# floswald/SMM.jl

Hardware: AMD Instinct MI355X
Metric: chain-evals/sec (whole node), serialNormal 2p/2m, 4096 chains x 200 iters (higher is better)
Workload: dtype f64

## Files before the change

### include/smmhip.h

```cpp
#ifndef SMMHIP_H
#define SMMHIP_H

#include <stdint.h>

#ifdef __cplusplus
extern "C" {
#endif

#define SMMHIP_ABI_VERSION 3

#define SMM_REDUCE_LANES 512

typedef enum {
    SMM_OK = 0,
    SMM_ERR_INVALID_ARG = -1,
    SMM_ERR_NO_DEVICE = -2,
    SMM_ERR_NEGATIVE_OBJECTIVE = -3,
    SMM_ERR_NO_DRAW_IN_SUPPORT = -4,
    SMM_ERR_BAD_BATCH = -5,
    SMM_ERR_MAXITER = -6,
    SMM_ERR_HIP = -7,
    SMM_ERR_STATE = -8,
    SMM_ERR_EXCHANGE_CAPACITY = -9
} smm_status_t;
// ... 382 lines not shown
typedef struct {
    double*  best;
    double*  value;
    double*  sim_moments;
    double*  simplex;
    double*  simplex_value;
    double*  size_x;
    double*  size_f;
    int32_t* iterations;
    int32_t* status;
    int32_t* moves;
    int32_t* n_eval;
    int64_t  evaluated;
} smm_opt_simplex_t;
int  smm_opt_simplex(void* ctx, const double* starts , int32_t K, double step, int32_t adaptive, double xatol, double fatol,
                     int32_t max_iter, smm_opt_simplex_t* out);

typedef struct {
    double*  best;
    double*  value;
    double*  sim_moments;
    double*  ssr;
    double*  grad;
    double*  jac;
    double*  lambda;
    double*  step;
    double*  dF;
    int32_t* active;
    int32_t* iterations;
    int32_t* tries;
    int32_t* n_eval;
    int32_t* status;
    int64_t  evaluated;
} smm_opt_lm_t;
int  smm_opt_lm(void* ctx, const double* starts , int32_t K, double fd_step, double lambda0, double lambda_up,
                double lambda_down, double xtol, double ftol, double gtol, int32_t max_iter, int32_t max_tries, smm_opt_lm_t* out);

typedef struct {
    double*  theta;
    double*  value;
    double*  sim_moments;
    double*  weight;
    double*  logw;
    int32_t* born;
    double*  eps;
    double*  p_acc;
    double*  gen_ess;
    int32_t* n_outside;
    int32_t* n_invalid;
    int32_t* n_underflow;
    int32_t* n_new_kept;
    double*  mean;
    double*  cov;
    double*  quantile;
    double   ess;
    int32_t  n_kept;
    int32_t  generations;
    int32_t  status;
    int32_t  reserved;
    int64_t  evaluated;
} smm_abc_pmc_t;
int  smm_abc_pmc(void* ctx, int32_t n_particles , int32_t n_keep , int32_t max_gen, double p_acc_min, double scale ,
                 double ridge, const double* probs, int32_t n_probs, smm_abc_pmc_t* out);

typedef struct {
    double*  mean;
    double*  var;
    double*  centre;
    double*  first;
    double*  total;
    double*  v_first;
    double*  v_total;
    double*  se_first;
    double*  se_total;
    int64_t  n_complete;
    int64_t  n_invalid;
    int64_t  evaluated;
} smm_sens_sobol_t;
int  smm_sens_sobol(void* ctx, int32_t n_base , const double* lo, const double* hi , smm_sens_sobol_t* out);
int  smm_get_timing(void* ctx, smm_timing_t* out);
int  smm_set_profiling(void* ctx, int32_t on);
int  smm_set_persistent(void* ctx, int32_t on);
int  smm_get_persistent(void* ctx, int32_t* available, int32_t* launches, int32_t* repairs);
int  smm_describe(void* ctx, char* out, int32_t cap);
int  smm_get_Z(void* ctx, double* Z);

#ifdef __cplusplus
}
#endif
#endif
```

### smm.jl_amd/_abi.py

```python
import ctypes as C
import os

import numpy as np

_HERE = os.path.dirname(os.path.abspath(__file__))
LIB_PATH = os.path.join(_HERE, "csrc", "libsmmhip.so")
HOOKS_LIB_PATH = os.path.join(_HERE, "csrc", "libsmmhip_hooks.so")

c_double_p = C.POINTER(C.c_double)
c_int32_p = C.POINTER(C.c_int32)
c_uint8_p = C.POINTER(C.c_uint8)
c_int8_p = C.POINTER(C.c_int8)

SMM_OK = 0
SMM_ERR_INVALID_ARG = -1
SMM_ERR_NO_DEVICE = -2
SMM_ERR_NEGATIVE_OBJECTIVE = -3
SMM_ERR_NO_DRAW_IN_SUPPORT = -4
SMM_ERR_BAD_BATCH = -5
SMM_ERR_MAXITER = -6
SMM_ERR_HIP = -7
SMM_ERR_STATE = -8
SMM_ERR_EXCHANGE_CAPACITY = -9

# ... 214 lines not shown
    ]


SYMBOLS = [
    ("smm_abi_version", C.c_int, []),
    ("smm_register_user_objective", C.c_int, [C.c_char_p, C.POINTER(C.c_int32)]),
    ("smm_register_user_objective_lanes", C.c_int, [C.c_char_p, C.c_int32, C.c_int32, C.POINTER(C.c_int32)]),
    ("smm_register_user_objective_rng", C.c_int, [C.c_char_p, C.c_int32, C.c_int32, C.POINTER(C.c_int32)]),
    ("smm_device_count", C.c_int, []),
    ("smm_ctx_create", C.c_int, [C.POINTER(smm_problem_t), C.POINTER(smm_bgp_opts_t), C.POINTER(smm_tables_t),
                                 C.POINTER(C.c_void_p)]),
    ("smm_ctx_destroy", None, [C.c_void_p]),
    ("smm_last_error", C.c_char_p, [C.c_void_p]),
    ("smm_bgp_step", C.c_int, [C.c_void_p, C.c_int32]),
    ("smm_bgp_step_async", C.c_int, [C.c_void_p, C.c_int32]),
    ("smm_sync", C.c_int, [C.c_void_p]),
    ("smm_bgp_local_step", C.c_int, [C.c_void_p]),
    ("smm_bgp_record_doubles", C.c_int, [C.c_void_p]),
    ("smm_bgp_export_records_dev", C.c_int, [C.c_void_p, C.c_void_p]),
    ("smm_bgp_exchange_dev", C.c_int, [C.c_void_p, C.c_void_p]),
    ("smm_bgp_a2a_capacity", C.c_int, [C.c_void_p]),
    ("smm_bgp_export_values_dev", C.c_int, [C.c_void_p, C.c_void_p]),
    ("smm_bgp_a2a_pack_dev", C.c_int, [C.c_void_p, C.c_void_p, C.c_void_p]),
    ("smm_bgp_a2a_apply_dev", C.c_int, [C.c_void_p, C.c_void_p]),
    ("smm_bgp_sharded_step", C.c_int, [C.c_void_p, C.c_void_p, C.c_void_p]),
    ("smm_bgp_sharded_finish", C.c_int, [C.c_void_p, C.c_void_p]),
    ("smm_bgp_p2p_init", C.c_int, [C.c_void_p, C.c_void_p, C.POINTER(C.c_void_p)]),
    ("smm_bgp_p2p_attach", C.c_int, [C.c_void_p, C.c_int32, C.c_void_p, C.c_void_p]),
    ("smm_bgp_p2p_step", C.c_int, [C.c_void_p, C.c_int32]),
    ("smm_bgp_p2p_finish", C.c_int, [C.c_void_p]),
    ("smm_stream", C.c_void_p, [C.c_void_p]),
    ("smm_eval_batch", C.c_int, [C.c_void_p, c_double_p, C.c_int32, c_double_p, c_double_p, c_int8_p]),
    ("smm_eval_batch_noseed", C.c_int, [C.c_void_p, c_double_p, C.c_int32, C.c_uint64, c_double_p, c_double_p, c_int8_p]),
    ("smm_get_history", C.c_int, [C.c_void_p, C.c_int32, C.c_int32, C.POINTER(smm_history_t)]),
    ("smm_get_chain_stats", C.c_int, [C.c_void_p, C.c_int32, C.c_int32, C.c_int32, c_double_p, C.c_int32,
                                      C.POINTER(smm_chain_stats_t)]),
    ("smm_get_chain_diag", C.c_int, [C.c_void_p, C.c_int32, C.c_int32, C.c_int32, C.c_int32, c_int32_p, C.c_int32,
                                     C.POINTER(smm_chain_diag_t)]),
    ("smm_get_group_stats", C.c_int, [C.c_void_p, C.c_int32, C.c_int32, C.c_int32, c_int32_p, C.c_int32, c_double_p, C.c_int32,
                                      C.POINTER(smm_group_stats_t)]),
    ("smm_get_histogram", C.c_int, [C.c_void_p, C.c_int32, C.c_int32, C.c_int32, c_int32_p, C.c_int32, C.c_int32, c_double_p, c_int32_p,
                                     C.c_int32, C.c_int32, C.POINTER(smm_histogram_t)]),
    ("smm_get_trace", C.c_int, [C.c_void_p, C.c_int32, C.c_int32, C.c_int32, C.c_int32, C.c_int32, c_int32_p, C.c_int32, c_double_p, C.c_int32,
                                C.POINTER(smm_trace_t)]),
    ("smm_get_rank_diag", C.c_int, [C.c_void_p, C.c_int32, C.c_int32, C.c_int32, C.c_int32, c_int32_p, C.c_int32,
                                    C.POINTER(smm_rank_diag_t)]),
    ("smm_get_draws", C.c_int, [C.c_void_p, C.c_int32, C.c_int32, C.c_int32, c_int32_p, C.c_int32, C.c_int32, C.c_int32, C.c_int64,
                                C.POINTER(smm_draws_t)]),
    ("smm_get_moment_stats", C.c_int, [C.c_void_p, C.c_int32, C.c_int32, C.c_int32, c_int32_p, C.c_int32, c_double_p, C.c_int32, C.c_double,
                                       C.POINTER(smm_moment_stats_t)]),
    ("smm_get_adjustment", C.c_int, [C.c_void_p, C.c_int32, C.c_int32, C.c_int32, c_int32_p, C.c_int32, C.c_double, C.c_int32, c_double_p,
                                     C.c_double, c_double_p, C.c_int32, C.POINTER(smm_adjustment_t)]),
    ("smm_get_reweighted", C.c_int, [C.c_void_p, C.c_int32, C.c_int32, C.c_int32, c_int32_p, C.c_int32, c_double_p, C.c_int32, c_double_p,
                                     C.c_int32, C.POINTER(smm_reweighted_t)]),
    ("smm_get_profile", C.c_int, [C.c_void_p, C.c_int32, C.c_int32, C.c_int32, c_int32_p, C.c_int32, C.c_int32, c_double_p, c_int32_p,
                                   C.c_int32, C.c_int32, C.POINTER(smm_profile_t)]),
    ("smm_get_density", C.c_int, [C.c_void_p, C.c_int32, C.c_int32, C.c_int32, c_int32_p, C.c_int32, c_double_p, C.c_int32, C.c_int32,
                                   c_double_p, c_double_p, C.POINTER(smm_density_t)]),
    ("smm_register_user_transform", C.c_int, [C.c_char_p, C.c_int32, C.POINTER(C.c_int32)]),
    ("smm_get_derived", C.c_int, [C.c_void_p, C.c_int32, C.c_int32, C.c_int32, C.c_int32, c_int32_p, C.c_int32, c_double_p, C.c_int32,
                                   c_double_p, C.c_int32, C.POINTER(smm_derived_t)]),
    ("smm_get_chain_cov", C.c_int, [C.c_void_p, C.c_int32, C.c_int32, C.c_int32, C.c_int32, c_int32_p, c_double_p, c_double_p]),
    ("smm_get_proposal", C.c_int, [C.c_void_p, c_double_p]),
    ("smm_set_proposal", C.c_int, [C.c_void_p, c_double_p]),
    ("smm_adapt_proposal", C.c_int, [C.c_void_p, C.c_int32, C.c_int32, C.c_int32, C.c_int32, C.c_int32, C.c_double, c_int32_p]),
    ("smm_get_state", C.c_int, [C.c_void_p, C.POINTER(smm_state_t)]),
    ("smm_set_state", C.c_int, [C.c_void_p, C.POINTER(smm_state_t), C.POINTER(smm_history_t)]),
    ("smm_set_population", C.c_int, [C.c_void_p, c_double_p, C.POINTER(smm_population_t)]),
    ("smm_scatter_population", C.c_int, [C.c_void_p, C.c_int32, C.c_double, C.c_int32, C.POINTER(smm_population_t)]),
    ("smm_opt_slices", C.c_int, [C.c_void_p, c_double_p, C.c_int32, C.c_int32, C.c_double, C.c_double, C.c_int32,
                                 C.POINTER(smm_opt_slices_t)]),
    ("smm_opt_simplex", C.c_int, [C.c_void_p, c_double_p, C.c_int32, C.c_double, C.c_int32, C.c_double, C.c_double, C.c_int32,
                                  C.POINTER(smm_opt_simplex_t)]),
    ("smm_opt_lm", C.c_int, [C.c_void_p, c_double_p, C.c_int32, C.c_double, C.c_double, C.c_double, C.c_double, C.c_double, C.c_double,
                             C.c_double, C.c_int32, C.c_int32, C.POINTER(smm_opt_lm_t)]),
    ("smm_abc_pmc", C.c_int, [C.c_void_p, C.c_int32, C.c_int32, C.c_int32, C.c_double, C.c_double, C.c_double, c_double_p, C.c_int32,
                              C.POINTER(smm_abc_pmc_t)]),
    ("smm_sens_sobol", C.c_int, [C.c_void_p, C.c_int32, c_double_p, c_double_p, C.POINTER(smm_sens_sobol_t)]),
    ("smm_get_timing", C.c_int, [C.c_void_p, C.POINTER(smm_timing_t)]),
    ("smm_get_Z", C.c_int, [C.c_void_p, c_double_p]),
    ("smm_set_profiling", C.c_int, [C.c_void_p, C.c_int32]),
    ("smm_set_persistent", C.c_int, [C.c_void_p, C.c_int32]),
    ("smm_get_persistent", C.c_int, [C.c_void_p, C.POINTER(C.c_int32), C.POINTER(C.c_int32), C.POINTER(C.c_int32)]),
    ("smm_describe", C.c_int, [C.c_void_p, C.c_char_p, C.c_int32]),
]


class SMMHipError(RuntimeError):
    def __init__(self, code, msg):
        super().__init__("smmhip error %d: %s" % (code, msg))
        self.code = code


def bind(lib, symbols=SYMBOLS, prefix_from="smm_", prefix_to=None):
    for name, res, args in symbols:
        n = name if prefix_to is None else prefix_to + name[len(prefix_from):]
        fn = getattr(lib, n)
        fn.restype = res
        fn.argtypes = args
    return lib


_lib = None


def load():
    global _lib
    if _lib is None:
        path = LIB_PATH
        if not os.path.exists(path):
            raise ImportError(
                "libsmmhip.so not found at %s — build it with `python -c 'import __graft_entry__ as g; g.build()'` "
                "(hipcc --offload-arch=gfx950). There is no CPU fallback." % path)
        _lib = bind(C.CDLL(path, mode=C.RTLD_GLOBAL))
        if _lib.smm_abi_version() != 3:
            raise ImportError("libsmmhip.so ABI version mismatch")
    return _lib


_hooks_lib = None


def load_hooks():
    global _hooks_lib
    if _hooks_lib is None:
        if not os.path.exists(HOOKS_LIB_PATH):
            raise ImportError("libsmmhip_hooks.so not found at %s — `make -C smm.jl_amd/csrc all`" % HOOKS_LIB_PATH)
        lib = bind(C.CDLL(HOOKS_LIB_PATH, mode=C.RTLD_GLOBAL))
        lib.smm_debug_has_test_hooks.restype = C.c_int
        if lib.smm_abi_version() != 3 or lib.smm_debug_has_test_hooks() != 1:
            raise ImportError("libsmmhip_hooks.so: wrong ABI version or built without -DSMM_TEST_HOOKS")
        lib.smm_debug_user_form.restype = C.c_int
        lib.smm_debug_user_form.argtypes = [C.c_int32, C.c_int, C.POINTER(C.c_ulonglong), C.POINTER(C.c_ulonglong), C.c_char_p, C.c_int]
        _hooks_lib = lib
    return _hooks_lib


def use_test_hooks(on=True):
    global _lib
    _lib = load_hooks() if on else None
    return load()


def dptr(a):
    return None if a is None else a.ctypes.data_as(c_double_p)


def f64(a, shape=None):
    a = np.ascontiguousarray(a, dtype=np.float64)
    if shape is not None:
        assert a.shape == tuple(shape), (a.shape, shape)
    return a


class HistoryBuffers:

    def __init__(self, nt, N, np_, nm):
        self.value = np.empty((nt, N)); self.prob = np.empty((nt, N))
        self.curr_val = np.empty((nt, N)); self.best_val = np.empty((nt, N))
        self.params = np.empty((nt, np_, N)); self.sim_moments = np.empty((nt, nm, N))
        self.best_id = np.empty((nt, N), np.int32); self.exchanged = np.empty((nt, N), np.int32)
        self.accepted = np.empty((nt, N), np.uint8); self.status = np.empty((nt, N), np.int8)

    FIELDS = ("value", "prob", "curr_val", "best_val", "params", "sim_moments", "best_id", "exchanged", "accepted",
              "status")

# ... 29 lines not shown
```

### smm.jl_amd/backend.py

```python
import builtins as _builtins
import ctypes as C

import numpy as np

from . import _abi as A


class Problem:

    def __init__(self, init, lb, ub, mom, w=None, ns=10000, objective_id=A.SMM_OBJ_NORM, obj_params=None):
        self.init = A.f64(init); self.lb = A.f64(lb); self.ub = A.f64(ub)
        self.mom = A.f64(mom)
        self.w = A.f64(np.full(len(self.mom), np.nan) if w is None else w)
        self.np = len(self.init); self.nm = len(self.mom); self.ns = int(ns)
        self.objective_id = int(objective_id)
        self.obj_params = None if obj_params is None else A.f64(obj_params)
        assert len(self.lb) == self.np and len(self.ub) == self.np and len(self.w) == self.nm

    def struct(self):
        p = A.smm_problem_t()
        p.np, p.nm, p.ns, p.objective_id = self.np, self.nm, self.ns, self.objective_id
        p.init, p.lb, p.ub, p.mom, p.w = map(A.dptr, (self.init, self.lb, self.ub, self.mom, self.w))
        p.obj_params = A.dptr(self.obj_params)
        p.n_obj_params = 0 if self.obj_params is None else len(self.obj_params)
# ... 529 lines not shown
                 converged=np.empty(K, np.int32))
        s = self._out(A.smm_opt_slices_t, r)
        self._check(self._fn("opt_slices")(self._ctx, A.dptr(st), K, int(npoints), float(tol), float("nan") if update is None else float(update),
                                           int(max_cycles), C.byref(s)))
        r["evaluated"] = int(s.evaluated)
        return r

    def opt_simplex(self, starts, step=0.05, adaptive=False, xatol=1e-4, fatol=1e-4, max_iter=None):
        st, K = self._opt_starts("opt_simplex", starts)
        V = self.np + 1
        r = dict(best=np.empty((self.np, K)), value=np.empty(K), sim_moments=np.empty((self.nm, K)), simplex=np.empty((V, self.np, K)),
                 simplex_value=np.empty((V, K)), size_x=np.empty(K), size_f=np.empty(K), iterations=np.empty(K, np.int32),
                 status=np.empty(K, np.int32), moves=np.empty((5, K), np.int32), n_eval=np.empty(K, np.int32))
        s = self._out(A.smm_opt_simplex_t, r)
        self._check(self._fn("opt_simplex")(self._ctx, A.dptr(st), K, float(step), int(bool(adaptive)), float(xatol), float(fatol),
                                            200 * self.np if max_iter is None else int(max_iter), C.byref(s)))
        r["evaluated"] = int(s.evaluated)
        return r

    def opt_lm(self, starts, fd_step=1e-4, lambda0=1e-3, lambda_up=10, lambda_down=10, xtol=1e-8, ftol=1e-12, gtol=0.0, max_iter=100,
               max_tries=12):
        st, K = self._opt_starts("opt_lm", starts)
        i32 = lambda *shape: np.empty(shape, np.int32)
        r = dict(best=np.empty((self.np, K)), value=np.empty(K), sim_moments=np.empty((self.nm, K)), ssr=np.empty(K), grad=np.empty((self.np, K)),
                 jac=np.empty((self.nm, self.np, K)), step=np.empty(K), dF=np.empty(K), active=i32(self.np, K), iterations=i32(K), tries=i32(K),
                 n_eval=i32(K), status=i32(K))
        r["lambda"] = np.empty(K)
        s = self._out(A.smm_opt_lm_t, r)
        self._check(self._fn("opt_lm")(self._ctx, A.dptr(st), K, float(fd_step), float(lambda0), float(lambda_up), float(lambda_down), float(xtol),
                                       float(ftol), float(gtol), int(max_iter), int(max_tries), C.byref(s)))
        r["evaluated"] = int(s.evaluated)
        return r

    def abc_pmc(self, n_particles, n_keep, max_gen=20, p_acc_min=0.05, scale=2.0, ridge=0.0, probs=()):
        Ap, G1 = max(int(n_keep), 0), max(int(max_gen), 0) + 1
        pr = A.f64(list(probs))
        r = dict(theta=np.empty((self.np, Ap)), value=np.empty(Ap), sim_moments=np.empty((self.nm, Ap)), weight=np.empty(Ap), logw=np.empty(Ap),
                 born=np.empty(Ap, np.int32), eps=np.empty(G1), p_acc=np.empty(G1), gen_ess=np.empty(G1), n_outside=np.empty(G1, np.int32),
                 n_invalid=np.empty(G1, np.int32), n_underflow=np.empty(G1, np.int32), n_new_kept=np.empty(G1, np.int32),
                 mean=np.empty(self.np), cov=np.empty((self.np, self.np)), quantile=np.empty((len(pr), self.np)))
        s = self._out(A.smm_abc_pmc_t, r)
        self._check(self._fn("abc_pmc")(self._ctx, int(n_particles), int(n_keep), int(max_gen), float(p_acc_min), float(scale), float(ridge),
                                        A.dptr(pr) if len(pr) else None, len(pr), C.byref(s)))
        for f in ("ess", "n_kept", "generations", "status", "evaluated"):
            r[f] = getattr(s, f)
        return r

    def sens_sobol(self, n_base, lo=None, hi=None):
        F = self.nm + 1
        box = [None if b is None else A.f64(list(np.asarray(b, float).reshape(-1))) for b in (lo, hi)]
        for b in box:
            if b is not None and len(b) != self.np:
                raise ValueError("sens_sobol: lo and hi take one entry per parameter")
        r = dict(mean=np.empty(F), var=np.empty(F), centre=np.empty(F))
        for f in ("first", "total", "v_first", "v_total", "se_first", "se_total"):
            r[f] = np.empty((F, self.np))
        s = self._out(A.smm_sens_sobol_t, r)
        self._check(self._fn("sens_sobol")(self._ctx, int(n_base), *[None if b is None else A.dptr(b) for b in box], C.byref(s)))
        for f in ("n_complete", "n_invalid", "evaluated"):
            r[f] = int(getattr(s, f))
        return r

    def timing(self):
        t = A.smm_timing_t()
        self._check(self._fn("get_timing")(self._ctx, C.byref(t)))
        return t

    def set_profiling(self, on=True):
        self._check(self._fn("set_profiling")(self._ctx, int(on)))

    def set_persistent(self, on=True):
        self._check(self._fn("set_persistent")(self._ctx, int(bool(on))))

    def describe(self):
        buf = C.create_string_buffer(256)
        self._check(self._fn("describe")(self._ctx, buf, 256))
        return dict(kv.split("=", 1) for kv in buf.value.decode().split())

    def persistent_info(self):
        a, l, r = C.c_int32(0), C.c_int32(0), C.c_int32(0)
        self._check(self._fn("get_persistent")(self._ctx, C.byref(a), C.byref(l), C.byref(r)))
        return bool(a.value), int(l.value), int(r.value)

    def Z(self):
        z = np.empty((self.nm, self.problem.ns))
        self._check(self._fn("get_Z")(self._ctx, A.dptr(z)))
        return z


def register_user_objective(source, n_sums=None, lanes=256, rng=False):
    lib = A.load()
    oid = C.c_int32(0)
    if rng:
        rc = lib.smm_register_user_objective_rng(source.encode(), 0 if n_sums is None else int(n_sums), int(lanes), C.byref(oid))
    elif n_sums is None:
        rc = lib.smm_register_user_objective(source.encode(), C.byref(oid))
    else:
        rc = lib.smm_register_user_objective_lanes(source.encode(), int(n_sums), int(lanes), C.byref(oid))
    if rc != 0:
        raise RuntimeError("smm_register_user_objective failed (%d): %s" % (rc, lib.smm_last_error(None).decode()))
    return int(oid.value)


class UserTransform:

    def __init__(self, source, n_out):
        self.source, self.n_out = source, int(n_out)
        self._handles = {}
        self.handle(A.load())

    def handle(self, lib):
        if id(lib) not in self._handles:
            tid = C.c_int32(-1)
            rc = lib.smm_register_user_transform(self.source.encode(), self.n_out, C.byref(tid))
            if rc != 0:
                raise A.SMMHipError(rc, "smm_register_user_transform failed: %s" % lib.smm_last_error(None).decode())
            self._handles[id(lib)] = int(tid.value)
        return self._handles[id(lib)]


def user_transform(source, n_out):
    return UserTransform(source, n_out)


def hip_context(problem, opts, tables=None):
    return BGPContext(problem, opts, tables)
```

### smm.jl_amd/csrc/smm_chain_persist_loc.hpp

```cpp
#pragma once
constexpr int PL_LOCN = NORM_CT + CONE_GCAP + 2;
constexpr uint32_t PL_PBASE = ((16u * PL_LOCN + 127u) & ~127u);
constexpr int PL_HASH = 1024;
constexpr size_t PL_TSW_BASE = (size_t)8 * 8192;
constexpr int PL_TSW_TILES = 2048, PL_TSW = 8;
constexpr size_t PL_LATE_BASE = PL_TSW_BASE + (size_t)PL_TSW_TILES * (NORM_WG / 64) * PL_TSW;
constexpr int PL_LATE_N = 16384;
static_assert(PL_LATE_BASE + PL_LATE_N <= (size_t)8 * 60000, "the stamp buffer: the exchange kernels' words start at 8 * 60000");

__host__ __device__ inline size_t persist_loc_smem_bytes(const int np) {
    const size_t hw = (size_t)((H_PARAMS + 2 * np + 1) & ~1);
    const size_t dbl = (size_t)NORM_CT * np + (size_t)np * 8 * NORM_CT + (size_t)NORM_CT * persist_line(np) + 2 * 64 * (size_t)(1 + 2 * np) +
                       2 * NORM_CT * hw + (size_t)PR_ZR * 64 + 16 + 16 + 2 * 64 * 2 + (size_t)PL_LOCN * np + (size_t)PL_LOCN +
                       (size_t)(NORM_WG / 64) * PL_TSW;
    return (size_t)PL_PBASE + 2 * (size_t)CONE_LEVELS * 64 * 4 + 2 * (size_t)CONE_GCAP * 2 + 4 * 16 * 4 + 2 * (size_t)PL_HASH * 4 + dbl * 8;
}

template <int NP>
struct PersistLocLds {
    using L = NormLayout<NP>;
    static constexpr int CT = NORM_CT, RW = L::RW, HW = L::HW, LW = PR_STW + RW, RNGW = 1 + 2 * NP;
    uint32_t pbase, gbase, hbase, tbase;
    uint32_t* s_hdr;
    double *s_theta, *s_part, *s_st, *s_rng, *s_hrow, *s_xrow, *s_z0, *s_const, *s_gth, *s_thr;
    uint4* s_donor;
    unsigned long long *s_ts, *s_wts;
    unsigned* s_arrived; int* s_minprog; unsigned* s_abort; unsigned* s_xmask; int* s_glready; int* s_pub; int* s_hready;
    __device__ inline PersistLocLds(unsigned char* lds) {
        pbase = PL_PBASE;
        gbase = pbase + 2u * CONE_LEVELS * 64 * 4;
        hbase = gbase + 2u * CONE_GCAP * 2;
        tbase = hbase + 4u * 16 * 4;
        s_hdr = (uint32_t*)(lds + hbase);
        s_theta = (double*)(lds + tbase + 2u * PL_HASH * 4);
        s_part = s_theta + CT * NP;
        s_st = s_part + NP * 8 * CT;
        s_rng = s_st + CT * LW;
        s_hrow = s_rng + 2 * 64 * RNGW;
        s_xrow = s_hrow + CT * HW;
        s_z0 = s_xrow + CT * HW;
        s_const = s_z0 + PR_ZR * 64;
        s_ts = (unsigned long long*)(s_const + 16);
        s_arrived = (unsigned*)(s_ts + 8);
        s_minprog = (int*)(s_arrived + 1);
        s_abort = s_arrived + 2;
        s_xmask = s_arrived + 3;
        s_glready = (int*)(s_arrived + 4);
        s_pub = (int*)(s_arrived + 5);
        s_hready = (int*)(s_arrived + 6);
        s_donor = (uint4*)(s_const + 16 + 16);
        s_gth = s_const + 16 + 16 + 2 * 64 * 2;
        s_thr = s_gth + PL_LOCN * NP;
        s_wts = (unsigned long long*)(s_thr + PL_LOCN);
    }
};

__device__ inline uint32_t pl_hslot(const uint32_t chain) { return (chain * 2654435761u) >> 22; }
static_assert(PL_HASH == 1024, "pl_hslot: 10 bits");
__device__ inline void pl_hash_put(uint32_t* tab, const uint32_t chain, const uint32_t local) {
    uint32_t h = pl_hslot(chain);
    while (atomicCAS(&tab[h], 0u, ((chain + 1u) << 16) | local) != 0u) h = (h + 1u) & (PL_HASH - 1);
}
__device__ inline uint32_t pl_hash_get(const uint32_t* tab, const uint32_t chain) {
    uint32_t h = pl_hslot(chain);
    for (int probe = 0; probe < PL_HASH; ++probe) {
        const uint32_t v = tab[h];
        if ((v >> 16) == chain + 1u) return v & 0xffffu;
        if (v == 0u) break;
        h = (h + 1u) & (PL_HASH - 1);
    }
    return 0xffffu;
}

__device__ inline void pl_wts_add(unsigned long long* w, const unsigned long long a, const unsigned long long b, const unsigned long long c,
                                  const unsigned long long d) {
    w[0] += a; w[1] += b; w[2] += c; w[3] += d; w[5] += 1ull;
}
__device__ inline void pl_wts_out(unsigned long long* ts, const unsigned long long* w, const int tile, const int wave) {
    if (tile >= PL_TSW_TILES) return;
    unsigned long long* o = ts + PL_TSW_BASE + ((size_t)tile * (NORM_WG / 64) + (size_t)wave) * PL_TSW;
    for (int k = 0; k < PL_TSW; ++k) o[k] = k == 4 ? (unsigned long long)__builtin_amdgcn_s_getreg((31 << 11) | 4) : w[k];
}

__device__ __attribute__((noinline, cold)) double pl_tie_value(const PrWait W, const unsigned char* win, const uint32_t o_rec, const int rel, const int rmask, const int Ng,
                                                               const uint32_t gl, const uint32_t c0g, const int RW, const int NPV, const int t, const uint32_t s) {
    const uint32_t g = s < (uint32_t)NORM_CT ? c0g + s : (uint32_t)*(const __attribute__((address_space(3))) uint16_t*)(size_t)(gl + 2u * (s - (uint32_t)NORM_CT));
    const uint4* ring = (const uint4*)(win + o_rec) + (size_t)((rel - 1) & rmask) * Ng * RW;
    return pr_tie_value(W, ring, nullptr, pr_tag32(W.epoch, rel - 1), RW, NPV, t, g);
}
struct PersistLocWalkValues {
    PrWait W; const unsigned char* win; uint32_t o_rec; int rel; int rmask; int Ng; uint32_t gl; uint32_t c0g; int RW; int NPV; int t;
    __device__ __forceinline__ double value(const uint32_t s) const { return pl_tie_value(W, win, o_rec, rel, rmask, Ng, gl, c0g, RW, NPV, t, s); }
};

struct PlGather3 { uint4 q0, q1, q2; };
__device__ __attribute__((noinline)) PlGather3 pl_wait_gather3(const PrWait W, const uint4* p0, const uint4* p1, const uint4* p2, const uint32_t tag, const int t, const int g) {
    PlGather3 o;
    o.q0 = make_uint4(0u, 0u, 0u, 0u); o.q1 = o.q0; o.q2 = o.q0;
    if (*W.s_abort) return o;
    const unsigned long long w0 = wall_clock64();
    unsigned spins = 0;
    for (;;) {
        __builtin_amdgcn_s_sleep(2);
        p2p_u32x4 q0, q1, q2;
        asm volatile("global_load_dwordx4 %0, %3, off sc0 sc1\n\tglobal_load_dwordx4 %1, %4, off sc0 sc1\n\tglobal_load_dwordx4 %2, %5, off sc0 sc1\n\ts_waitcnt vmcnt(0)"
                     : "=&v"(q0), "=&v"(q1), "=&v"(q2) : "v"(p0), "v"(p1), "v"(p2) : "memory");
        o.q0 = make_uint4(q0.x, q0.y, q0.z, q0.w); o.q1 = make_uint4(q1.x, q1.y, q1.z, q1.w); o.q2 = make_uint4(q2.x, q2.y, q2.z, q2.w);
        if (p2p_ll_ok(o.q0, tag) && p2p_ll_ok(o.q1, tag) && p2p_ll_ok(o.q2, tag)) break;
        if ((++spins & 63u) == 0u && pr_give_up(W, w0)) { pr_abort(W, t, g); break; }
    }
    return o;
}

template <int NP, bool WIDE, bool SH, bool PCT = false>
__global__ __launch_bounds__(NORM_WG, 4) void k_chain_persist_loc(const PersistArgs A) {
    static_assert(!PCT || (WIDE && !SH), "thresholds by chain: the wide walk of a single shard");
    static_assert(NP == 1 || NP == 2, "one moment per half of the workgroup");
    extern __shared__ __attribute__((aligned(16))) unsigned char lds[];
    using LY = PersistLocLds<NP>;
    constexpr int CT = NORM_CT, RW = LY::RW, HW = LY::HW, LW = LY::LW, RNGW = LY::RNGW;
    constexpr int NPC = RW / 2, NPH = HW / 2;
    constexpr uint32_t SB = WIDE ? 16u : 8u;
    const int tid = (int)threadIdx.x, lane = tid & 63;
    const int wave = __builtin_amdgcn_readfirstlane(tid >> 6);
    const int tile = (int)blockIdx.x, tiles = (int)gridDim.x;
    const int N = A.N;
    const LY Y(lds);
    const uint32_t epoch = A.epoch;
    const int t0 = A.t0, t1 = A.t1;
    unsigned char* const mine = A.self;
    uint32_t* const pr_ctl = (uint32_t*)(mine + A.o_ctl);
    uint32_t* const pr_progress = (uint32_t*)(mine + A.o_progress);
    const PrWait W{A.err, pr_ctl, Y.s_abort, A.epoch, A.tmo};
    const int rmask = A.ring_k - 1;
    const int tiles_all = SH ? tiles * A.G : tiles;
    const uint32_t c0g = (uint32_t)(A.offset + tile * CT);
    const bool exch_any = A.Ng > 1;
    auto exch_on = [&](const int tx) { return exch_any && tx >= A.exch_from; };

    if (error_before(*(const volatile unsigned long long*)A.err, t0)) return;

    if (tid < 64) {
        const int cl = lane >> 2, r = lane & 3, c = tile * CT + cl;
        if (c < N) {
            const double2* g_cs = (const double2*)(A.cs + (size_t)c * CSW);
            const double2* g_rec = (const double2*)(A.rec_in + (size_t)c * RW);
            double2* st2 = (double2*)(Y.s_st + cl * LW);
            for (int i = r; i < 6; i += 4) st2[i] = g_cs[i];
            for (int i = r; i < NPC; i += 4) st2[PR_STW / 2 + i] = g_rec[i];
            if (r == 0) {
                const double v0 = g_rec[0].x;
                if (SH && v0 != v0) pr_report(A.err, 3, t0, (int)c0g + cl);
                if constexpr (WIDE) ((uint4*)lds)[cl] = make_uint4((uint32_t)__double2loint(v0), (uint32_t)__double2hiint(v0), (uint32_t)cl, 0u);
                else ((uint2*)lds)[cl] = make_uint2(order_key32(v0), (uint32_t)cl);
                for (int k = 0; k < NP; ++k) Y.s_gth[cl * NP + k] = A.rec_in[(size_t)c * RW + 3 + k];
                if constexpr (PCT) Y.s_thr[cl] = A.mi_g[c0g + (uint32_t)cl];
            }
        }
#pragma unroll
        for (int u = 0; u < PR_ZR; ++u) Y.s_z0[u * 64 + lane] = (lane + u * WG < A.ns) ? A.Z[lane + (size_t)u * WG] : 0.0;
    }
    if (tid >= 64 && tid < 64 + NP) {
        const int k = tid - 64;
        Y.s_const[k] = A.lb[k]; Y.s_const[NP + k] = A.ub[k]; Y.s_const[2 * NP + k] = A.mom[k]; Y.s_const[3 * NP + k] = A.w[k];
    }
    if (tid == 128) {
        Y.s_const[4 * NP] = A.failbox ? A.objp[0] : 1.0; Y.s_const[4 * NP + 1] = A.failbox ? A.objp[1] : 0.0;
        Y.s_const[4 * NP + 2] = (double)A.ns;
        *Y.s_arrived = 0u; *Y.s_minprog = 0; *Y.s_abort = 0u; *Y.s_xmask = 0u; *Y.s_glready = t0 - 2; *Y.s_pub = t0 - 2; *Y.s_hready = t0 - 2;
    }
    if (tid >= 192 && tid < 200) Y.s_ts[tid - 192] = 0ull;
    if (A.ts && tid >= 256 && tid < 256 + (NORM_WG / 64) * PL_TSW) Y.s_wts[tid - 256] = 0ull;
    if (wave == 3 && lane < CONE_HDRW) {
        if (A.walk_first) Y.s_hdr[((t0 - 1) & 3) * 16 + lane] = A.cone_hdr[((size_t)(t0 - 1 - A.plan_t0) * tiles + tile) * CONE_HDRW + lane];
        if (t0 < t1 && exch_on(t0)) Y.s_hdr[(t0 & 3) * 16 + lane] = A.cone_hdr[((size_t)(t0 - A.plan_t0) * tiles + tile) * CONE_HDRW + lane];
    }
    if constexpr (SH) {
        if (tile == 0 && wave == 2 && lane < A.G) {
            unsigned char* w = nullptr;
#pragma unroll
            for (int p = 0; p < P2P_MAXG; ++p) w = lane == p ? A.win[p] : w;
            __hip_atomic_store((uint32_t*)(w + A.o_arrive + 128 * (size_t)A.rank), epoch, __ATOMIC_RELAXED, __HIP_MEMORY_SCOPE_SYSTEM);
        }
        if (wave == 2) {
            const unsigned long long w0 = wall_clock64();
            unsigned spins = 0;
            bool there = lane >= A.G;
            while (__ballot(!there) != 0ull) {
                if (!there) there = (int)(__hip_atomic_load((const uint32_t*)(mine + A.o_arrive + 128 * (size_t)lane), __ATOMIC_RELAXED, __HIP_MEMORY_SCOPE_SYSTEM) - epoch) >= 0;
                if ((++spins & 63u) == 0u && (wall_clock64() - w0 > A.tmo)) {
                    if (lane == 0) { pr_report(A.err, 3, t0, (int)c0g); __hip_atomic_store(pr_ctl, epoch, __ATOMIC_RELAXED, __HIP_MEMORY_SCOPE_SYSTEM); }
                    break;
                }
                __builtin_amdgcn_s_sleep(2);
            }
        }
    }
    PR_BARRIER();
    if (tid == 0 && SH && pr_load4_sys(pr_ctl) == epoch) *Y.s_abort = 1u;
    auto request_lists = [&](const int tx) {
        const size_t tb = (size_t)(tx - A.plan_t0) * tiles + tile;
        const uint32_t hw1 = Y.s_hdr[(tx & 3) * 16];
        const int nsub1 = (int)(hw1 & 0xffffu), ngat1 = (int)(hw1 >> 16);
        const uint32_t b = (uint32_t)(tx & 1);
        if (wave >= 8 && 4 * (wave - 8) < nsub1)
            lds_dma16((const uint4*)(A.cone_pairs + tb * (CONE_LEVELS * 64)) + (tid - 512), Y.pbase + b * (CONE_LEVELS * 64 * 4) + (uint32_t)(wave - 8) * 1024u);
        if (wave == 3 && 8 * lane < ngat1)
            lds_dma16((const uint4*)(A.cone_gather + tb * CONE_GCAP) + lane, Y.gbase + b * (CONE_GCAP * 2));
    };
    auto build_table = [&](const int tx, const int lane) {
        const int ngat = (int)(Y.s_hdr[(tx & 3) * 16] >> 16);
        if (!A.tables_local) {
            uint32_t* tab = (uint32_t*)(lds + Y.tbase) + (tx & 1) * PL_HASH;
            for (int x = lane; x < PL_HASH / 4; x += 64) ((uint4*)tab)[x] = make_uint4(0u, 0u, 0u, 0u);
            asm volatile("s_waitcnt lgkmcnt(0)" ::: "memory");
            const uint16_t* gl = (const uint16_t*)(lds + Y.gbase) + (tx & 1) * CONE_GCAP;
            for (int e = lane; e < ngat; e += 64) pl_hash_put(tab, (uint32_t)gl[e], (uint32_t)(CT + e));
            asm volatile("s_waitcnt lgkmcnt(0)" ::: "memory");
        }
    };
    auto fix_lists = [&](const int tx, const int t_report, const int lane) {
        const uint32_t* hd = Y.s_hdr + (tx & 3) * 16;
        const int nsub1 = (int)(hd[0] & 0xffffu);
// ... 119 lines not shown
        if (wave == 0) {
            const int cl = lane >> 2, r = lane & 3, c = tile * CT + cl;
            if (c < N) {
                double nr[RW];
#pragma unroll
                for (int f = 0; f < RW; ++f) nr[f] = Y.s_st[cl * LW + PR_STW + f];
                publish(0, (int)c0g + cl, r, nr);
            }
        }
        PR_BARRIER();
        if (wave >= 8) fix_lists(t0 - 1, t0, lane);
        if (wave >= 4 && wave < 8) gather(t0 - 1, 0, t0, tid);
    }

    if (wave != 0) {
        const int h = wave >> 3, wih = wave & 7;
        const bool simw = h < NP;
        const bool rng_here = A.rb == nullptr;
        double z[PR_ZR];
        int nfull = 0;
        bool extra = false;
        if (simw) {
            const int l = wih * 64 + lane;
            const double* zr = A.Z + (size_t)h * A.zstride + l;
#pragma unroll
            for (int u = 0; u < PR_ZR; ++u) z[u] = (l + u * WG < A.ns) ? zr[(size_t)u * WG] : 0.0;
            nfull = A.ns / WG;
            extra = l < A.ns - nfull * WG;
        } else {
#pragma unroll
            for (int u = 0; u < PR_ZR; ++u) z[u] = 0.0;
        }
        auto make_rng = [&](const int tn, const int batch) {
            const int c1 = tile * CT + (lane >> 2);
            if (c1 >= N) return;
            const uint32_t g1 = c0g + (uint32_t)(lane >> 2);
            double* o = Y.s_rng + ((tn & 1) * 64 + lane) * RNGW;
            if (rng_here) {
                if (batch == 0) o[0] = rng_u(A.seed, g1, (uint32_t)tn);
                uint32_t tr = (uint32_t)(batch * NORM_NR + (lane & 3));
                asm volatile("" : "+v"(tr));
#pragma unroll
                for (int q = 0; 2 * q < NP; ++q) {
                    double z0, z1;
                    rng_prop_normal2(A.seed, g1, (uint32_t)tn, tr, (uint32_t)q, z0, z1);
                    o[1 + batch * NP + 2 * q] = z0;
                    if (2 * q + 1 < NP) o[1 + batch * NP + 2 * q + 1] = z1;
                }
            } else if (batch == 0) {
                const double* g_rb = A.rb + ((size_t)(tn - A.rb_t0) * N + c1) * A.RBW;
                const int rr = lane & 3;
                o[0] = g_rb[0];
#pragma unroll
                for (int k = 0; k < NP; ++k) {
                    o[1 + k] = rr < A.rb_tries ? g_rb[1 + rr * NP + k] : 0.0;
                    o[1 + NP + k] = NORM_NR + rr < A.rb_tries ? g_rb[1 + (NORM_NR + rr) * NP + k] : 0.0;
                }
            }
        };
        auto store_rows = [&](const double* s_row, const int trow, const unsigned mask) {
            for (int e = lane; e < CT * NPH; e += 64) {
                const int cl = e / NPH, i = e - cl * NPH, c = tile * CT + cl;
                if (c < N && ((mask >> cl) & 1u)) ((double2*)(A.hrec + ((size_t)(trow - 1) * N + c) * HW))[i] = ((const double2*)(s_row + cl * HW))[i];
            }
        };
        if (wave == 1 || (wave == 2 && PR_AHEAD > 1)) make_rng(t0, wave - 1);
        for (int t = t0; t <= t1; ++t) {
            const int rel = t - t0 + 1;
            PR_BARRIER();
            uint32_t nhdr = 0u;
            const bool want_hdr = wave == 3 && lane < CONE_HDRW && t + 1 < t1 && exch_on(t + 1);
            if (wave == 3) {
                if (t > t0) {
                    store_rows(Y.s_hrow, t - 1, 0xffffu);
                    store_rows(Y.s_xrow, t - 2, *Y.s_xmask);
                }
                if (want_hdr) nhdr = A.cone_hdr[((size_t)(t + 1 - A.plan_t0) * tiles + tile) * CONE_HDRW + lane];
            }
            if (t < t1 && exch_on(t)) request_lists(t);
            PR_BARRIER();
            unsigned long long tw0 = 0, tw1 = 0, tw2 = 0;
            if (A.ts) tw0 = wall_clock64();
            if (simw) {
                __builtin_amdgcn_s_setprio(1);
                if (nfull == PR_ZR - 1) persist_simulate<NP, true>(z, nfull, extra, Y.s_theta, Y.s_part, h, wih, A.ts != nullptr, tw1);
                else persist_simulate<NP, false>(z, nfull, extra, Y.s_theta, Y.s_part, h, wih, A.ts != nullptr, tw1);
                if (A.ts) tw2 = wall_clock64();
                __builtin_amdgcn_fence(__ATOMIC_RELEASE, "workgroup");
                const int lane3 = (int)__builtin_amdgcn_mbcnt_hi(~0u, __builtin_amdgcn_mbcnt_lo(~0u, 0u));
                if (lane3 == 0) __hip_atomic_fetch_add(Y.s_arrived, 1u, __ATOMIC_RELAXED, __HIP_MEMORY_SCOPE_WORKGROUP);
                __builtin_amdgcn_s_setprio(0);
            }
            const int lane = (int)__builtin_amdgcn_mbcnt_hi(~0u, __builtin_amdgcn_mbcnt_lo(~0u, 0u));
            const bool lists = t < t1 && exch_on(t);
            if (wave == 3 || wave >= 8) {
                if (wave == 3 && want_hdr) Y.s_hdr[((t + 1) & 3) * 16 + lane] = nhdr;
                asm volatile("s_waitcnt vmcnt(0)" ::: "memory");
                if (wave == 3 && lane == 0) __hip_atomic_store(Y.s_glready, t, __ATOMIC_RELEASE, __HIP_MEMORY_SCOPE_WORKGROUP);
                if (wave == 3 && lists) {
                    build_table(t, lane);
                    if (lane == 0) __hip_atomic_store(Y.s_hready, t, __ATOMIC_RELEASE, __HIP_MEMORY_SCOPE_WORKGROUP);
                }
                if (wave >= 8 && lists) {
                    if (!A.tables_local) while (__hip_atomic_load(Y.s_hready, __ATOMIC_ACQUIRE, __HIP_MEMORY_SCOPE_WORKGROUP) != t) __builtin_amdgcn_s_sleep(1);
                    fix_lists(t, t + 1, lane);
                }
            }
            if (wave == 2) {
                const int m = pr_min_progress(pr_progress, epoch, tiles_all, lane);
                if (lane == 0) {
                    __hip_atomic_store(Y.s_minprog, m, __ATOMIC_RELAXED, __HIP_MEMORY_SCOPE_WORKGROUP);
                    if (pr_load4_sys(pr_ctl) == epoch) *Y.s_abort = 1u;
                    if (lists && A.cone_ok[t - A.plan_t0] == 0u) pr_report(A.err, 3, t + 1, (int)c0g);
                }
                if constexpr (SH) {
                    if (*Y.s_abort && lane < A.G) {
                        unsigned char* w = nullptr;
#pragma unroll
                        for (int p = 0; p < P2P_MAXG; ++p) w = lane == p ? A.win[p] : w;
                        __hip_atomic_store((uint32_t*)(w + A.o_ctl), epoch, __ATOMIC_RELAXED, __HIP_MEMORY_SCOPE_SYSTEM);
                    }
                }
            }
            if (wave == 2 && PR_AHEAD > 1 && rng_here && t < t1) {
                const unsigned want = (unsigned)(8 * NP) * (unsigned)rel;
                while (__hip_atomic_load(Y.s_arrived, __ATOMIC_RELAXED, __HIP_MEMORY_SCOPE_WORKGROUP) < want) __builtin_amdgcn_s_sleep(2);
            }
            if ((wave == 1 || (wave == 2 && PR_AHEAD > 1)) && t < t1) make_rng(t + 1, wave - 1);
            if (wave >= 4 && wave < 8 && lists) {
                while (__hip_atomic_load(Y.s_glready, __ATOMIC_ACQUIRE, __HIP_MEMORY_SCOPE_WORKGROUP) != t) __builtin_amdgcn_s_sleep(1);
                while (__hip_atomic_load(Y.s_pub, __ATOMIC_RELAXED, __HIP_MEMORY_SCOPE_WORKGROUP) != t) __builtin_amdgcn_s_sleep(1);
                __builtin_amdgcn_s_sleep(PR_GATHER_DELAY);
                gather(t, rel, t + 1, wave * 64 + lane);
            }
            if (A.ts && lane == 0) pl_wts_add(Y.s_wts + wave * PL_TSW, tw0, tw1, tw2, wall_clock64());
        }
        PR_BARRIER();
        if (A.ts && lane == 0) pl_wts_out(A.ts, Y.s_wts + wave * PL_TSW, tile, wave);
        if (wave == 3) { store_rows(Y.s_hrow, t1, 0xffffu); store_rows(Y.s_xrow, t1 - 1, *Y.s_xmask); }
        if (wave == 1) {
            const int cl = lane >> 2, r = lane & 3, c = tile * CT + cl;
            if (c < N) {
                const double2* st2 = (const double2*)(Y.s_st + cl * LW);
                double2* g_cs = (double2*)(A.cs + (size_t)c * CSW);
                for (int i = r; i < 6; i += 4) g_cs[i] = i == 2 ? make_double2(st2[2].x, 0.0) : st2[i];
                for (int i = r; i < NPC; i += 4) ((double2*)(A.rec_out + (size_t)c * RW))[i] = st2[PR_STW / 2 + i];
                if (r == 0) {
                    const double v = Y.s_st[cl * LW + PR_STW];
                    A.vals_out[c] = v;
                    if (A.slot8_out) { A.slot8_out[c] = make_uint2(order_key32(v), (uint32_t)c); if (v != v) atomicOr(A.walk_flags, 1u); }
                }
            }
        }
        return;
    }

    const int nfull0 = A.ns / WG;
    for (int t = t0; t <= t1; ++t) {
        const int rel = t - t0 + 1;
        const bool exch = t == t0 ? A.walk_first != 0 : exch_on(t - 1);
        double z0[PR_ZR];
        uint32_t wmeta;
        PR_BARRIER();
        {
            const int lane = (int)__builtin_amdgcn_mbcnt_hi(~0u, __builtin_amdgcn_mbcnt_lo(~0u, 0u));
            const int cl = lane >> 2, r = lane & 3;
            const int c = tile * CT + cl;
            const bool valid = c < N;
            double* st = Y.s_st + cl * LW;
            unsigned long long ts1 = 0;
            if (A.ts && lane == 0) { ts1 = wall_clock64(); if (t != t0) Y.s_ts[0] += ts1 - Y.s_ts[7]; }
            wmeta = (uint32_t)cl;
            if (exch) {
                const uint32_t lbase = Y.pbase + (uint32_t)((t - 1) & 1) * (CONE_LEVELS * 64 * 4);
// ... 52 lines not shown
                    bool ok = !found;
#pragma unroll
                    for (int k = 0; k < NP; ++k) {
                        const double step = sigma * o[1 + NP + k];
                        x[k] = mu01[k] + step;
                        if (!(x[k] >= 0.0 && x[k] <= 1.0)) ok = false;
                    }
                    if (NORM_NR + r >= A.smpl_iters || (A.user_n && NORM_NR + r >= A.rb_tries)) ok = false;
                    const unsigned long long m = __ballot(ok);
                    const unsigned quad = (unsigned)(m >> (lane & ~3)) & 0xfu;
                    if (!found && quad) {
                        const int rwin = __builtin_ctz(quad);
#pragma unroll
                        for (int k = 0; k < NP; ++k) {
                            const double lbk = Y.s_const[k];
                            const double sc = x[k] * (Y.s_const[NP + k] - lbk);
                            const double thk = sc + lbk;
                            th[k] = quad_bcast_dyn(thk, lane, rwin);
                        }
                        found = true;
                    }
                    j_next = 2 * NORM_NR;
                }
                if (__any(!found)) {
                    const PrTries TR{A.rb, A.seed, A.rb_t0, A.N, A.RBW, A.rb_tries, A.user_n, A.smpl_iters, A.offset};
                    const PrTh<NP> lt = persist_late_tries<NP>(TR, o, t, c, valid, lane, found, sigma, mu01[0], mu01[NP - 1], Y.s_const, th[0], th[NP - 1], j_next);
#pragma unroll
                    for (int k = 0; k < NP; ++k) th[k] = lt.th[k];
                    found = lt.found;
                    if (!found && r == 0) pr_report(A.err, ERRK_NO_DRAW, t, (int)c0g + cl);
                }
                if (A.ts && lane == 0) {
                    Y.s_wts[6] += 1ull; Y.s_wts[7] += wall_clock64();
                    atomicAdd(A.ts + PL_LATE_BASE + (size_t)(t & (PL_LATE_N - 1)), 1ull);
                }
            }
            if (r == 0) {
#pragma unroll
                for (int k = 0; k < NP; ++k) Y.s_theta[cl * NP + k] = th[k];
            }
            if (A.ts && lane == 0) {
                const unsigned long long ts4 = wall_clock64();
                Y.s_ts[1] += ts2 - ts1; Y.s_ts[3] += ts4 - ts2; Y.s_ts[6] = ts4;
            }
        }
        PR_BARRIER();
        unsigned long long tw0 = 0, tw1 = 0, tw2 = 0, tw3 = 0;
        if (A.ts) tw0 = wall_clock64();
        {
            const int lane_a = (int)__builtin_amdgcn_mbcnt_hi(~0u, __builtin_amdgcn_mbcnt_lo(~0u, 0u));
            const bool extra0 = lane_a < A.ns - nfull0 * WG;
#pragma unroll
            for (int u = 0; u < PR_ZR; ++u) z0[u] = Y.s_z0[u * 64 + lane_a];
            {
                const int cl = lane_a >> 2, r = lane_a & 3;
                const bool valid = tile * CT + cl < N;
                const uint32_t src = wmeta & 0xffffu;
                const uint32_t lbase = Y.pbase + (uint32_t)((t - 1) & 1) * (CONE_LEVELS * 64 * 4);
                const uint16_t* gl = (const uint16_t*)(lds + Y.gbase) + ((t - 1) & 1) * CONE_GCAP;
                int partner = 0;
                if (wmeta >> 16) {
                    const uint32_t pl = lean_partner<0, WIDE ? 4 : 3>(lds, lbase, wmeta, (uint32_t)cl) - 1u;
                    partner = 1 + (int)(pl < (uint32_t)CT ? c0g + pl : (uint32_t)gl[pl - CT]);
                }
                if (valid && src != (uint32_t)cl) {
                    const uint32_t src_g = src < (uint32_t)CT ? c0g + src : (uint32_t)gl[src - CT];
                    const unsigned char* dwin = mine;
                    if constexpr (SH) {
                        const int owner = (int)src_g / A.N;
#pragma unroll
                        for (int p = 0; p < P2P_MAXG; ++p) dwin = owner == p ? A.win[p] : dwin;
                    }
                    const uint4* g_ll = (const uint4*)(dwin + A.o_rec) + ((size_t)((rel - 1) & rmask) * A.Ng + src_g) * RW;
                    const uint32_t dbase = (uint32_t)((unsigned char*)Y.s_donor - lds);
                    pr_dma16(g_ll + r, dbase);
                    if (4 + r < RW) pr_dma16(g_ll + 4 + r, dbase + 64 * 16);
                }
                if (r == 0) {
                    double* st = Y.s_st + cl * LW;
                    st[CS_PARTNER] = (double)partner;
                    st[CS_WASX] = (double)src;
                }
            }
            __builtin_amdgcn_s_setprio(1);
            if (nfull0 == PR_ZR - 1) persist_simulate<NP, true>(z0, nfull0, extra0, Y.s_theta, Y.s_part, 0, 0, A.ts != nullptr, tw1);
            else persist_simulate<NP, false>(z0, nfull0, extra0, Y.s_theta, Y.s_part, 0, 0, A.ts != nullptr, tw1);
            if (A.ts) tw2 = wall_clock64();
            __builtin_amdgcn_fence(__ATOMIC_RELEASE, "workgroup");
            if (lane_a == 0) __hip_atomic_fetch_add(Y.s_arrived, 1u, __ATOMIC_RELAXED, __HIP_MEMORY_SCOPE_WORKGROUP);
            __builtin_amdgcn_s_setprio(0);
        }
        {
            const unsigned want = (unsigned)(8 * NP) * (unsigned)rel;
            while (__hip_atomic_load(Y.s_arrived, __ATOMIC_RELAXED, __HIP_MEMORY_SCOPE_WORKGROUP) < want) __builtin_amdgcn_s_sleep(1);
            __builtin_amdgcn_fence(__ATOMIC_ACQUIRE, "workgroup");
        }
        if (A.ts) tw3 = wall_clock64();
        const int lane = (int)__builtin_amdgcn_mbcnt_hi(~0u, __builtin_amdgcn_mbcnt_lo(~0u, 0u));
        const int cl = lane >> 2, r = lane & 3;
        const int c = tile * CT + cl;
        const bool valid = c < N;
        double* st = Y.s_st + cl * LW;
        unsigned long long ts5 = 0;
        if (A.ts && lane == 0) ts5 = wall_clock64();
        if (valid) {
            const int src = (int)st[CS_WASX];
            const bool donor = src != cl;
            double rc2[RW];
#pragma unroll
            for (int f = 0; f < RW; ++f) rc2[f] = st[PR_STW + f];
            if (donor) {
                asm volatile("s_waitcnt vmcnt(0)" ::: "memory");
                const uint32_t tag = pr_tag32(epoch, rel - 1);
                double rr[8];
#pragma unroll
                for (int f = 0; f < 8; ++f) rr[f] = 0.0;
                bool ok = true;
#pragma unroll
                for (int f = 0; f < RW; ++f) {
                    const uint4 q = Y.s_donor[(f >> 2) * 64 + 4 * cl + (f & 3)];
                    ok = ok && p2p_ll_ok(q, tag);
                    rr[f] = p2p_ll_double(q);
                }
                if (__builtin_expect(!ok, 0)) {
                    const uint16_t* gl = (const uint16_t*)(lds + Y.gbase) + ((t - 1) & 1) * CONE_GCAP;
                    const uint32_t src_g = (uint32_t)src < (uint32_t)CT ? c0g + (uint32_t)src : (uint32_t)gl[src - CT];
                    const unsigned char* dwin = mine;
                    if constexpr (SH) {
                        const int owner = (int)src_g / A.N;
#pragma unroll
                        for (int p = 0; p < P2P_MAXG; ++p) dwin = owner == p ? A.win[p] : dwin;
                    }
                    const uint4* g_ll = (const uint4*)(dwin + A.o_rec) + ((size_t)((rel - 1) & rmask) * A.Ng + src_g) * RW;
#pragma unroll
                    for (int f = 0; f < RW; f += 2) {
                        const PrLL2 w2 = pr_wait_ll2(W, g_ll + f, g_ll + f + 1, tag, t, (int)c0g + cl);
                        rr[f] = p2p_ll_double(w2.q0); rr[f + 1] = p2p_ll_double(w2.q1);
                    }
                }
#pragma unroll
                for (int f = 0; f < RW; ++f) rc2[f] = rr[pr_ring_index<NP>(f)];
            }
            if (lane == 0) announce(rel);
            const double atun = st[CS_ATUN];
            const double uu = Y.s_rng[((t & 1) * 64 + lane) * RNGW];
            double th2[NP], sm[NP];
#pragma unroll
            for (int k = 0; k < NP; ++k) th2[k] = Y.s_theta[cl * NP + k];
            double value;
            int status;
            norm_quad_finish<NP>(in_failbox(th2[0], Y.s_const + 4 * NP), r, Y.s_part + cl, Y.s_const[4 * NP + 2],
                                 Y.s_const + 2 * NP, Y.s_const + 3 * NP, sm, value, status);
            const double old = rc2[0];
            const AcceptDecision d = accept_decide(false, status, value, old, atun, uu, pr_exp);
            if (d.negative && r == 0) pr_report(A.err, ERRK_NEGATIVE, t, (int)c0g + cl);
            const double prob = d.prob;
            const bool acc = d.acc;
            status = d.status;
            const double accd = acc ? 1.0 : 0.0;
            const double v = acc ? value : old;
            double nr[RW];
            record_head(nr, rc2, acc, value, prob, status);
#pragma unroll
            for (int k = 0; k < NP; ++k) { nr[3 + k] = acc ? th2[k] : rc2[3 + k]; nr[3 + NP + k] = acc ? sm[k] : rc2[3 + NP + k]; }
            if (RW > 3 + 2 * NP) nr[RW - 1] = 0.0;
            if (t < t1) {
                if (__builtin_expect(rel > rmask && __hip_atomic_load(Y.s_minprog, __ATOMIC_RELAXED, __HIP_MEMORY_SCOPE_WORKGROUP) < rel - rmask, 0))
                    pr_wait_progress(W, pr_progress, Y.s_minprog, rel - rmask, tiles_all, lane, t, (int)c0g + cl);
#ifdef SMM_TEST_HOOKS
                if (tile == A.slow_tile) { const unsigned long long w0 = wall_clock64(); while (wall_clock64() - w0 < (unsigned long long)A.slow_ticks) __builtin_amdgcn_s_sleep(8); }
#endif
                publish(rel, (int)c0g + cl, r, nr);
                if (lane == 0) __hip_atomic_store(Y.s_pub, t, __ATOMIC_RELAXED, __HIP_MEMORY_SCOPE_WORKGROUP);
// ... 62 lines not shown
```

### smm.jl_amd/csrc/smm_create_host.hpp

```cpp
#pragma once

namespace {

int persist_occupancy(Ctx* c, const Forms& F, int objective_id) {
    if (F.persist_user || (F.persist == PERSIST_TILE && c->obj == SMM_OBJ_USER)) {
        const UserForm form = user_form_wanted(F, c->has_chol);
        {
            std::lock_guard<std::mutex> lock(g_user_mutex);
            UserObjective& u = g_user_objectives[objective_id - SMM_OBJ_USER_BASE];
            if (!user_form_compile(u, form)) {
                if (getenv("SMMHIP_VERBOSE"))
                    fprintf(stderr, "libsmmhip: the persistent form of this user objective is not available:\n%s\n", u.form[form].log.c_str());
                return 0;
            }
            HIPCHK(hipModuleLoadData(&c->pmod, u.form[form].code.data()));
        }
        HIPCHK(hipModuleGetFunction(&c->pfn, c->pmod, user_form_kernel(form)));
    }
    const PersistKernel K = persist_kernel(c, F);
    int per_cu = 0;
    if (K.mfn) {
        (void)hipFuncSetAttribute((const void*)K.mfn, hipFuncAttributeMaxDynamicSharedMemorySize, (int)K.smem);
        (void)hipGetLastError();
        HIPCHK(hipModuleOccupancyMaxActiveBlocksPerMultiprocessor(&per_cu, K.mfn, K.block.x, K.smem));
// ... 157 lines not shown
    for (int wv = 0; wv < 8; ++wv)
        for (int s = 0; s < DENSE_D / 4; ++s)
            for (int l = 0; l < 64; ++l)
                for (int tt = 0; tt < 2; ++tt) {
                    const int j = 16 * (2 * wv + tt) + (l & 15), d = 4 * s + (l >> 4);
                    A2f[(((size_t)wv * (DENSE_D / 4) + s) * 64 + l) * 2 + tt] = M[nB + (size_t)j * DENSE_D + d];
                }
}
void upload_inputs(Ctx* c, const smm_problem_t* prob, const smm_bgp_opts_t* opts, const smm_tables_t* tab) {
    KParams& P = c->P;
    const size_t N = (size_t)P.N, TN = (size_t)P.T * P.N;
    HIPCHK(hipSetDevice(c->device));
    HIPCHK(hipStreamCreateWithFlags(&c->stream, hipStreamNonBlocking));
    HIPCHK(hipEventCreate(&c->ev0));
    HIPCHK(hipEventCreate(&c->ev1));
    (void)hipDeviceGetAttribute(&c->dev.n_cus, hipDeviceAttributeMultiprocessorCount, c->device);
    const char* tsv = getenv("SMMHIP_TS");
    if (tsv && (tsv[0] == '1' || tsv[0] == '2')) P.ts = dalloc<unsigned long long>(c, (size_t)8 * 65536);
    P.ts_levels = tsv && tsv[0] == '2';
    P.init = dupload(c, prob->init, P.np); P.lb = dupload(c, prob->lb, P.np); P.ub = dupload(c, prob->ub, P.np);
    P.mom = dupload(c, prob->mom, P.nm); P.w = dupload(c, prob->w, P.nm);
    P.objp = prob->n_obj_params > 0 ? dupload(c, prob->obj_params, prob->n_obj_params) : nullptr;
    if (c->obj == SMM_OBJ_USER) {
        {
            std::lock_guard<std::mutex> lock(g_user_mutex);
            HIPCHK(hipModuleLoadData(&c->umod, g_user_objectives[prob->objective_id - SMM_OBJ_USER_BASE].code.data()));
        }
        HIPCHK(hipModuleGetFunction(&c->ufn, c->umod, "smm_user_eval_kernel"));
        if (c->u_rng) HIPCHK(hipModuleGetFunction(&c->ufn_noseed, c->umod, "smm_user_eval_noseed_kernel"));
        P.u_theta = dalloc<double>(c, N * P.np); P.u_simM = dalloc<double>(c, N * P.nm);
        P.u_value = dalloc<double>(c, N); P.u_status = dalloc<int>(c, N);
    }
    if (c->obj == SMM_OBJ_DENSE) {
        const size_t nB = (size_t)DENSE_D * P.np;
        std::vector<double> M(nB + (c->dense2 ? (size_t)DENSE_D * DENSE_D : 0) + (size_t)P.nm * DENSE_D);
        if (prob->n_obj_params) memcpy(M.data(), prob->obj_params, M.size() * 8);
        else {
            for (size_t i = 0; i < M.size(); i += 2) {
                double z0, z1;
                box_muller(philox_stream(P.seed, 5, (uint32_t)(i >> 1), (uint32_t)((i >> 1) >> 32), 0, 0), z0, z1);
                M[i] = z0 / sqrt(i < nB ? (double)P.np : (double)DENSE_D);
                if (i + 1 < M.size()) M[i + 1] = z1 / sqrt(i + 1 < nB ? (double)P.np : (double)DENSE_D);
            }
        }
        std::vector<double> Bf, Af, A2f;
        dense_operands(M, P.np, P.nm, c->dense2, Bf, Af, A2f);
        P.dense_Bf = dupload(c, Bf.data(), Bf.size());
        P.dense_Af = dupload(c, Af.data(), Af.size());
        if (c->dense2) P.dense_A2f = dupload(c, A2f.data(), A2f.size());
    }
    const int rows = (P.ns + WG - 1) / WG;
    P.zstride = ((rows + ZU) / ZU) * ZU * WG;
    std::vector<double> Z((size_t)P.nm * P.zstride, 0.0);
    for (int k = 0; k < P.nm; ++k)
        for (int s = 0; s < P.ns; ++s)
            Z[(size_t)k * P.zstride + s] = (tab && tab->Z) ? tab->Z[(size_t)k * P.ns + s] : rng_Z(P.seed, (uint32_t)k, (uint32_t)s);
    P.Z = dupload(c, Z.data(), Z.size());
    P.min_improve_g = dupload(c, opts->min_improve, P.Ng);
    if (c->has_chol) P.chol_L = dupload(c, opts->chol_L, (size_t)(P.chol_per_chain ? P.Ng : 1) * P.np * P.np);
    if (c->has_utab) P.user_utab = dupload(c, tab->probs_acc, TN);
    if (c->has_ntab) P.user_ntab = dupload(c, tab->prop_normals, TN * (size_t)tab->prop_tries * P.np);
    if (P.n_pairs_tab > 0) P.pairtab = dupload(c, tab->pairs, (size_t)P.T * tab->n_pairs * 2);
}

void choose_forms(Ctx* c, int objective_id, bool ask = true, int per_cu = -1) {
    KParams& P = c->P;
    Forms& F = c->F;
    F = select_forms(c, c->H, c->dev);
    if (F.persist != PERSIST_NONE && (ask || per_cu >= 0)) {
        c->dev.per_cu = ask ? persist_occupancy(c, F, objective_id) : per_cu;
        F = select_forms(c, c->H, c->dev);
    }
    P.tile_off = F.tile_off;
    P.gen_lean = F.gen_keys ? 2 : F.gen_lean ? 1 : 0;
    P.rows_cap = F.rows_cap;
    if (F.lean_plan) {
        P.lean_wide = F.lean_wide ? 1 : 0;
        P.plan_Kp = lean_walk_Kp(P.plan_K);
        P.lean_unit = F.lean_wide ? LeanLayout<LEAN_WIDE>::unit(P.Ng) : LeanLayout<LEAN_KEYS>::unit(P.Ng);
    }
    if (F.cone_tiles) { P.cone_tiles = F.cone_tiles; P.cone_ct = F.cone_ct; }
}

void alloc_windows(Ctx* c) {
    KParams& P = c->P;
    const Forms& F = c->F;
    const size_t N = (size_t)P.N, Ng = (size_t)P.Ng, K = (size_t)P.plan_K, W = (size_t)F.plan_cap;
    c->win_rb = dalloc<double>(c, (size_t)F.win_cap * N * P.RBW);
    HIPCHK(hipMemset(c->win_rb, 0, (size_t)F.win_cap * N * P.RBW * 8));
    if (F.plan != PLAN_NONE) alloc_level_tables(c, c->win, F.xk == XK_ROWS, (size_t)F.cone_tiles, F.cone_gather);
    P.cone_ok = c->win.cone_ok; P.cone_hdr = c->win.cone_hdr; P.cone_pairs = c->win.cone_pairs; P.cone_gather = c->win.cone_gather;
    if (F.plan == PLAN_BIG) c->big_scratch = dalloc<uint32_t>(c, W * BigPlanScratch::words(P.Ng, P.plan_K));
    if (F.xk == XK_ROWS) {
        c->slots17 = dalloc<uint32_t>(c, Ng + 4);
        c->nan_flags = dalloc<uint32_t>(c, 4);
        HIPCHK(hipMemset(c->nan_flags, 0, 16));
    }
    if (F.plan == PLAN_LDS) {
        c->win_plan = dalloc<unsigned long long>(c, W * K);
        c->win_plan_mi = dalloc<double>(c, W * K);
    }
    if (F.lean_plan) {
        c->win_lv_pairs_p = dalloc<uint32_t>(c, W * P.plan_Kp + 512);
        c->win_lv_offp = dalloc<uint32_t>(c, W * LV_OFFP);
    }
    if (F.walk_slots) {
        for (int b = 0; b < 2; ++b) c->slot8_buf[b] = dalloc<uint2>(c, N + 4 + 128);
        P.slot8 = c->slot8_buf[0];
        P.walk_flags = dalloc<uint32_t>(c, 4);
        HIPCHK(hipMemset(P.walk_flags, 0, 16));
    }
    if (F.cone_big || F.persist_sh_big) c->cb_scratch = dalloc<uint32_t>(c, W * cone_big_scratch_words(P.Ng, P.plan_K));
    if (F.plan_ahead) {
        HIPCHK(hipStreamCreateWithFlags(&c->pstream, hipStreamNonBlocking));
        HIPCHK(hipEventCreateWithFlags(&c->ev_free, hipEventDisableTiming));
        static_cast<LevelTables&>(c->ps[0]) = c->win;
        alloc_level_tables(c, c->ps[1], true, (size_t)F.cone_tiles, true);
        for (Ctx::PlanSet& S : c->ps) {
            HIPCHK(hipHostMalloc((void**)&S.ok_host, W * 4, hipHostMallocDefault));
            HIPCHK(hipEventCreateWithFlags(&S.done, hipEventDisableTiming));
        }
    }
}

void init_state(Ctx* c, const smm_bgp_opts_t* opts) {
    KParams& P = c->P;
    const int N = P.N, Ng = P.Ng, T = P.T;
    std::vector<double> cs((size_t)N * CSW, 0.0);
    for (int i = 0; i < N; ++i) {
        double* b = cs.data() + (size_t)i * CSW;
        b[CS_SIGMA] = opts->sigma[opts->chain_offset + i];
        b[CS_BEST] = INFINITY; b[CS_BESTID] = -1.0; b[CS_BESTP] = INFINITY; b[CS_BESTPID] = -1.0;
        b[CS_ATUN] = opts->acc_tuner[opts->chain_offset + i];
    }
    P.cs = dupload(c, cs.data(), cs.size());
    std::vector<double> rec((size_t)N * P.RW, 0.0);
    for (int i = 0; i < N; ++i) rec[(size_t)i * P.RW] = INFINITY;
    for (int b = 0; b < 2; ++b) c->rec[b] = dupload(c, rec.data(), rec.size());
    P.xres = dalloc<unsigned long long>(c, Ng);
    if (N > 0 && Ng % N == 0 && opts->chain_offset % N == 0) {
        c->a2a_G = Ng / N;
        c->a2a_cap = c->H.a2a_cap ? c->H.a2a_cap : a2a_capacity(N, c->a2a_G);
        c->a2a_send_idx = dalloc<int32_t>(c, (size_t)c->a2a_G * c->a2a_cap);
        c->a2a_send_cnt = dalloc<int32_t>(c, (size_t)c->a2a_G);
        c->a2a_rowidx = dalloc<int32_t>(c, (size_t)N);
    }
    for (int b = 0; b < 2; ++b) c->vals_buf[b] = dalloc<double>(c, (size_t)N + 4);
    P.vals = c->vals_buf[0];
    if (c->F.plan != PLAN_LDS) {
        const int Kmax = std::max(P.plan_K, 1);
        P.xval = dalloc<double>(c, Ng); P.xnext = dalloc<int32_t>(c, Ng); P.xpairs = dalloc<int32_t>(c, (size_t)Kmax * 2);
        P.xsrc = dalloc<int32_t>(c, Ng); P.xpartner = dalloc<int32_t>(c, Ng);
        P.xslot = dalloc<double>(c, (size_t)Ng * 2);
    }
    std::vector<double> row((size_t)N * P.HW, NAN);
    for (int i = 0; i < N; ++i) history_head(row.data() + (size_t)i * P.HW, NAN, NAN, INFINITY, INFINITY, -1.0, 0.0, 0.0, 0.0);
    P.hrec = dalloc<double>(c, (size_t)T * N * P.HW);
    HIPCHK(hipMemcpy(P.hrec, row.data(), row.size() * 8, hipMemcpyHostToDevice));
    for (size_t have = 1; have < (size_t)T; have *= 2) {
        const size_t n = std::min(have, (size_t)T - have);
        HIPCHK(hipMemcpy(P.hrec + have * N * P.HW, P.hrec, n * N * P.HW * 8, hipMemcpyDeviceToDevice));
    }
    P.err = dalloc<unsigned long long>(c, 1);
    const unsigned long long e = ERR_NONE;
    HIPCHK(hipMemcpy(P.err, &e, 8, hipMemcpyHostToDevice));
}

void lds_limits(Ctx* c) {
    const Forms& F = c->F;
    const bool on[] = {F.plan == PLAN_BIG, F.xk == XK_ROWS || F.xk == XK_KEY, F.plan == PLAN_LDS, F.cone_big};
    for (int id = 0; id < XI_COUNT; ++id) {
        const ExchInstance I = exch_instance(id, c->P.Ng);
        if (I.fn && I.cap && on[I.group]) HIPCHK(hipFuncSetAttribute(I.fn, hipFuncAttributeMaxDynamicSharedMemorySize, (int)I.cap));
    }
    for (int family = 0; family < EF_COUNT; ++family)
        for (int kind = 0; kind < 3; ++kind) HIPCHK(hipFuncSetAttribute(eval_instance(family, kind).fn, hipFuncAttributeMaxDynamicSharedMemorySize, (int)LDS_CU));
    for (int family = 0; family < CF_COUNT; ++family)
        for (int np = 1; np <= 4; ++np)
            for (int b = 0; b < 2; ++b) HIPCHK(hipFuncSetAttribute(chain_instance(family, np, b != 0).fn, hipFuncAttributeMaxDynamicSharedMemorySize, (int)LDS_CU));
    if (tile_smem(c, F, is_sim(c->obj) ? F.ct : (c->obj == SMM_OBJ_DENSE ? 16 : 8)) > LDS_CU) throw std::string("tile does not fit the 160 KiB LDS");
}

#ifdef SMM_TEST_HOOKS
std::string forms_line(const Ctx* c, const DeviceFacts& dev) {
    std::string s = describe_text(c);
    const Forms& F = c->F;
    auto add = [&s](const char* name, long long v) { s += std::string(" ") + name + "=" + std::to_string(v); };
#define FIELD(f) add("F." #f, (long long)F.f)
    FIELD(plan); FIELD(xk); FIELD(rows_cap); FIELD(lean_plan); FIELD(lean_wide); FIELD(plan_ahead); FIELD(win_cap); FIELD(plan_cap);
    FIELD(ct); FIELD(norm_fast); FIELD(norm_narrow); FIELD(tpw); FIELD(tile_off);
    FIELD(inline_walk); FIELD(gen_lean); FIELD(gen_keys); FIELD(dense_keys); FIELD(cone); FIELD(cone_big); FIELD(walk_slots);
    FIELD(cone_tiles); FIELD(cone_ct); FIELD(cone_gather);
    FIELD(persist); FIELD(persist_wide); FIELD(persist_sh); FIELD(persist_sh_big); FIELD(persist_user); FIELD(max_tiles); FIELD(defer_resolve);
#undef FIELD
    add("n_cus", dev.n_cus); add("per_cu", dev.per_cu);
    return s;
}
#endif

}

extern "C" {

void smm_ctx_destroy(void* ctx) {
    Ctx* c = (Ctx*)ctx;
    if (!c) return;
    (void)hipSetDevice(c->device);
    if (c->stream) (void)hipStreamSynchronize(c->stream);
    if (c->pstream) { (void)hipStreamSynchronize(c->pstream); (void)hipStreamDestroy(c->pstream); }
    if (c->ev_free) (void)hipEventDestroy(c->ev_free);
    for (Ctx::PlanSet& S : c->ps) { if (S.done) (void)hipEventDestroy(S.done); if (S.ok_host) (void)hipHostFree(S.ok_host); }
    for (void* p : c->allocs) (void)hipFree(p);
    for (void* w : c->p2p_opened) if (w) (void)hipIpcCloseMemHandle(w);
    if (c->p2p_mine) (void)hipFree(c->p2p_mine);
    if (c->st_scr) (void)hipFree(c->st_scr);
    if (c->red_res) (void)hipFree(c->red_res);
    if (c->umod) (void)hipModuleUnload(c->umod);
    if (c->pmod) (void)hipModuleUnload(c->pmod);
    for (const auto& tm : c->tmods) (void)hipModuleUnload(tm.second);
    if (c->ev0) (void)hipEventDestroy(c->ev0);
    if (c->ev1) (void)hipEventDestroy(c->ev1);
    for (hipEvent_t e : c->pev) (void)hipEventDestroy(e);
    if (c->stream) (void)hipStreamDestroy(c->stream);
    delete c;
}

int smm_ctx_create(const smm_problem_t* prob, const smm_bgp_opts_t* opts, const smm_tables_t* tab, void** out) {
    if (const int rc = check_create_args(prob, opts, tab, out)) return rc;
    int ndev = 0;
    if (hipGetDeviceCount(&ndev) != hipSuccess || ndev < 1)
        return fail(nullptr, SMM_ERR_NO_DEVICE, "no HIP device available: libsmmhip has no CPU fallback");
    if (opts->device < 0 || opts->device >= ndev) return fail(nullptr, SMM_ERR_INVALID_ARG, "bad device ordinal");
    Ctx* c = new Ctx();
    try {
        c->H = read_hooks();
        if (const char* why = create_facts(c, prob, opts, tab)) throw std::string(why);
        upload_inputs(c, prob, opts, tab);
        choose_forms(c, prob->objective_id);
        alloc_windows(c);
        init_state(c, opts);
        if (c->F.persist != PERSIST_NONE) alloc_persist(c);
        lds_limits(c);
        reducer_kernel_attributes();
        HIPCHK(hipDeviceSynchronize());
    } catch (const std::string& m) {
        g_create_err = m;
        smm_ctx_destroy(c);
        return SMM_ERR_HIP;
    }
    *out = c;
    return SMM_OK;
}

int smm_describe(void* ctx, char* out, int32_t cap) {
    Ctx* c = (Ctx*)ctx;
    if (!c || !out || cap < 1) return SMM_ERR_INVALID_ARG;
    snprintf(out, (size_t)cap, "%s", describe_text(c).c_str());
    return SMM_OK;
}

#ifdef SMM_TEST_HOOKS
int smm_debug_forms(void* ctx, const smm_problem_t* prob, const smm_bgp_opts_t* opts, const smm_tables_t* tab, int n_cus, int per_cu, char* out, int cap) {
    if (!out || cap < 1) return SMM_ERR_INVALID_ARG;
    std::string line;
    if (ctx) {
        const Ctx* c = (Ctx*)ctx;
        line = forms_line(c, c->dev);
    } else {
        void* none = nullptr;
        if (const int rc = check_create_args(prob, opts, tab, &none)) return rc;
        Ctx c;
        c.H = read_hooks();
        if (const char* why = create_facts(&c, prob, opts, tab)) return fail(nullptr, SMM_ERR_HIP, why);
        c.dev = DeviceFacts{n_cus, -1};
        choose_forms(&c, 0, false, per_cu);
        line = forms_line(&c, c.dev);
    }
    snprintf(out, (size_t)cap, "%s", line.c_str());
    return SMM_OK;
}
#endif

}
```

### smm.jl_amd/csrc/smm_launch_host.hpp

```cpp
#pragma once

namespace {

int exchange_K(const Ctx* c) { return c->P.n_pairs_tab > 0 ? c->P.n_pairs_tab : n_exchange_pairs(c->P.Ng); }
bool exchange_active(const Ctx* c, int t) { return t >= c->exchange_from && c->P.Ng > 1; }

ExchInstance exch_instance(int id, int Ng = 0);
template <class... Args>
void launch_exch(Ctx* c, int id, dim3 grid, size_t smem, hipStream_t st, const Args&... args) {
    const ExchInstance I = exch_instance(id);
    if (!I.fn) throw std::string("exchange kernel ") + I.name + " is not part of this build";
    void* a[] = {(void*)&args...};
    launch_fn(c, I.fn, grid, dim3(I.block), smem, st, a, I.stamped);
}
size_t plan_smem(int Ng, int K, bool cones) { return cones ? std::max(plan_lds_bytes(Ng, K), plan_cone_bytes()) : plan_lds_bytes(Ng, K); }
void launch_plan_big(Ctx* c, const KParams& P, int t, int W, const LevelTables& L, hipStream_t st, bool cones) {
    launch_exch(c, XI_PLAN_BIG, dim3(W), plan_big_lds_bytes(P.Ng), st, P, t, c->big_scratch, L.lv_pairs, L.lv_mi, L.lv_off, L.lv_rows, L.lv_rowinfo);
    if (!cones) return;
    launch_exch(c, XI_CONE_CHAINS, dim3(W), cone_chains_lds_bytes(P.Ng), st, P, (const uint32_t*)L.lv_pairs, (const uint32_t*)L.lv_off, c->cb_scratch);
    const unsigned blocks = ((P.cone_tiles + CONEB_WAVES - 1) / CONEB_WAVES) * ((W + 7) & ~7);
    launch_exch(c, XI_CONE_TILES, dim3(blocks), cone_tiles_lds_bytes(P.plan_K), st, P, W, (const uint32_t*)c->cb_scratch);
}
void point_tables(KParams& P, const LevelTables& L) {
    P.lv_pairs = L.lv_pairs; P.lv_mi = L.lv_mi; P.lv_off = L.lv_off; P.lv_rows = L.lv_rows; P.lv_rowinfo = L.lv_rowinfo;
    P.cone_ok = L.cone_ok; P.cone_hdr = L.cone_hdr; P.cone_pairs = L.cone_pairs; P.cone_gather = L.cone_gather;
}
void plan_window_into(Ctx* c, int k, int t) {
    Ctx::PlanSet& S = c->ps[k];
    KParams Pw = c->P;
    HIPCHK(hipEventRecord(c->ev_free, c->stream));
    HIPCHK(hipStreamWaitEvent(c->pstream, c->ev_free, 0));
    point_tables(Pw, S);
    const int W = std::min(c->F.plan_cap, Pw.T - t + 1);
    launch_plan_big(c, Pw, t, W, S, c->pstream, true);
    HIPCHK(hipMemcpyAsync(S.ok_host, S.cone_ok, (size_t)W * 4, hipMemcpyDeviceToHost, c->pstream));
    HIPCHK(hipEventRecord(S.done, c->pstream));
    S.t0 = t; S.w = W;
}

bool plan_ahead_covers(const Ctx* c, int t) {
    const Ctx::PlanSet& S = c->ps[c->ps_act ^ 1];
    return c->F.plan_ahead && S.w >= 2 && S.t0 == t - 1;
}

void ensure_windows(Ctx* c, int t, bool rng = true) {
    KParams& P = c->P;
    const bool pregen = rng && !(c->F.norm_fast && !P.user_ntab && !P.user_utab);
    if (pregen && !(t >= c->rng_t0 && t < c->rng_t0 + c->rng_w)) {
        int W = std::min(c->F.win_cap, P.T - t + 1);
        if ((c->F.persist == PERSIST_GEN || c->F.persist == PERSIST_TILE) && c->persist_on && !c->persist_broken && !c->in_repair && !P.user_ntab && !P.user_utab &&
            c->persist_launches != c->pregen_seen_launches) W = std::min(W, 2);
        c->pregen_seen_launches = c->persist_launches;
        const size_t Q = (size_t)(P.np + 1) / 2;
        const size_t per_iter = (size_t)P.rb_tries * Q * P.N;
        hipLaunchKernelGGL(k_pregen_rng, dim3((unsigned)((per_iter + 255) / 256), (unsigned)W), dim3(256), 0, c->stream, P, t, W, c->win_rb);
        c->rng_t0 = t; c->rng_w = W;
        P.rb = c->win_rb; P.rb_t0 = t;
    }
    if (c->F.plan_ahead && !(t >= c->plan_t0 && t < c->plan_t0 + c->plan_w)) {
        const int nx = c->ps_act ^ 1;
        Ctx::PlanSet& S = c->ps[nx];
        if (!(S.w > 0 && (S.t0 == t || (S.t0 == t - 1 && S.w >= 2)))) plan_window_into(c, nx, t);
        HIPCHK(hipEventSynchronize(S.done));
        HIPCHK(hipStreamWaitEvent(c->stream, S.done, 0));
        c->ps_act = nx; c->plan_t0 = S.t0; c->plan_w = S.w;
        P.plan_t0 = S.t0;
        point_tables(P, S);
        c->cone_big_ok.assign(S.ok_host, S.ok_host + S.w);
        c->ps[nx ^ 1].w = 0;
        if (S.t0 + S.w <= P.T) plan_window_into(c, nx ^ 1, S.t0 + S.w - (S.w >= 2 && c->F.plan_cap >= 2 ? 1 : 0));
    }
    if (c->F.plan == PLAN_BIG && !c->F.plan_ahead && !(t >= c->plan_t0 && t < c->plan_t0 + c->plan_w)) {
        const int W = std::min(c->F.plan_cap, P.T - t + 1);
        launch_plan_big(c, P, t, W, c->win, c->stream, c->F.cone_big || c->F.persist_sh_big);
        c->plan_t0 = t; c->plan_w = W;
        P.plan_t0 = t;
        if (c->F.cone_big) {
            c->cone_big_ok.resize((size_t)W);
            HIPCHK(hipMemcpyAsync(c->cone_big_ok.data(), P.cone_ok, (size_t)W * 4, hipMemcpyDeviceToHost, c->stream));
            HIPCHK(hipStreamSynchronize(c->stream));
        }
        point_tables(P, c->win);
    }
    if (c->F.plan == PLAN_LDS && P.Ng > 1 && !(t >= c->plan_t0 && t < c->plan_t0 + c->plan_w)) {
        const int W = std::min(c->F.plan_cap, P.T - t + 1);
        launch_exch(c, XI_PLAN, dim3(W), plan_smem(P.Ng, P.plan_K, c->F.cone || c->F.persist != PERSIST_NONE), c->stream, P, t, c->win_plan, c->win_plan_mi,
                    c->win.lv_pairs, c->win.lv_mi, c->win.lv_off, c->win_lv_pairs_p, c->win_lv_offp);
        c->plan_t0 = t; c->plan_w = W;
        P.plan = c->win_plan; P.plan_mi = c->win_plan_mi; P.plan_t0 = t;
        point_tables(P, c->win);
        P.lv_pairs_p = c->win_lv_pairs_p; P.lv_offp = c->win_lv_offp;
    }
}

enum ChainFamily {
    CF_SIM, CF_SIM_2, CF_DENSE, CF_GEN_KEYS, CF_GEN_64, CF_GEN_2, CF_GEN,
    CF_NORM_NARROW_CONE, CF_NORM_ANY, CF_NORM_WIDE, CF_NORM_NARROW,
    CF_NORM,
    CF_P2P_ROWS_NARROW, CF_P2P_ROWS,
    CF_P2P,
    CF_COUNT
};
template <class F>
const void* by_np(int np, F f) {
    switch (np) {
        case 1: return f(std::integral_constant<int, 1>{});
        case 2: return f(std::integral_constant<int, 2>{});
        case 3: return f(std::integral_constant<int, 3>{});
        default: return f(std::integral_constant<int, 4>{});
    }
}
ChainKernel chain_instance(int family, int np, bool b) {
#define ITER(KIND, CT, TPW, NAME) \
    ChainKernel{b ? (const void*)k_chain_iter<KIND, CT, TPW, true> : (const void*)k_chain_iter<KIND, CT, TPW, false>, NAME, WG * TPW, CT, TPW}
#define NORM(KERN, NAME, BLOCK) ChainKernel{by_np(np, [](auto NP) { return (const void*)KERN<decltype(NP)::value>; }), NAME, BLOCK, NORM_CT, 1}
#define NORM_B(KERN, NAME) \
    ChainKernel{by_np(np, [b](auto NP) { return !b ? (const void*)KERN<decltype(NP)::value, false> : (const void*)KERN<decltype(NP)::value, true>; }), NAME, NORM_WG, NORM_CT, 1}
    switch (family) {
        case CF_SIM: return ITER(1, 8, 1, "iter<sim,8>");
        case CF_SIM_2: return ITER(1, 8, 2, "iter<sim,8,2>");
        case CF_DENSE: return ITER(2, 16, 1, "iter<dense,16>");
        case CF_GEN_KEYS: return ITER(0, 16, 2, "iter<gen,16,2>");
        case CF_GEN_64: return ITER(0, 64, 1, "iter<gen,8>");
        case CF_GEN_2: return ITER(0, 8, 2, "iter<gen,8,2>");
        case CF_GEN: return ITER(0, 8, 1, "iter<gen,8>");
        case CF_NORM_NARROW_CONE: return NORM(k_chain_iter_norm_narrow_cone, "iter_norm_narrow_cone", NORM_WG / 2);
        case CF_NORM_ANY: return NORM(k_chain_iter_norm_any, "iter_norm_any", NORM_WG);
        case CF_NORM_WIDE: return NORM(k_chain_iter_norm_wide, "iter_norm_wide", NORM_WG);
        case CF_NORM_NARROW: return NORM(k_chain_iter_norm_narrow, "iter_norm_narrow", NORM_WG / 2);
        case CF_NORM: return NORM_B(k_chain_iter_norm, "iter_norm");
        case CF_P2P_ROWS_NARROW: return NORM(k_chain_iter_norm_p2p_rows_narrow, "iter_norm_p2p_rows_narrow", NORM_WG / 2);
        case CF_P2P_ROWS: return NORM(k_chain_iter_norm_p2p_rows, "iter_norm_p2p_rows", NORM_WG);
        default: return NORM_B(k_chain_iter_norm_p2p, "iter_norm_p2p");
    }
#undef ITER
#undef NORM
#undef NORM_B
}
ChainKernel chain_kernel(const Ctx* c, int flags) {
    const KParams& P = c->P;
    const Forms& F = c->F;
    const bool walk = (flags & F_WALK_INLINE) != 0, user = c->obj == SMM_OBJ_USER;
    if (F.norm_fast && !user) {
        if (walk && F.cone_big) return chain_instance(CF_NORM_NARROW_CONE, P.np, false);
        if (walk && (!F.lean_plan || c->deep_plan || c->nan_values || P.mi_pct)) return chain_instance(CF_NORM_ANY, P.np, false);
        if (walk && P.lean_wide) return chain_instance(CF_NORM_WIDE, P.np, false);
        if (!walk && F.norm_narrow) return chain_instance(CF_NORM_NARROW, P.np, false);
        return chain_instance(CF_NORM, P.np, walk);
    }
    const bool fits64 = tile_smem_base(c, 64) <= (size_t)60 * 1024;
    const int family = is_sim(c->obj) ? (F.tpw == 2 ? CF_SIM_2 : CF_SIM) : c->obj == SMM_OBJ_DENSE ? CF_DENSE : user ? (fits64 ? CF_GEN_64 : CF_GEN)
                     : F.gen_keys ? CF_GEN_KEYS : (fits64 && !F.inline_walk) ? CF_GEN_64 : F.tpw == 2 ? CF_GEN_2 : CF_GEN;
    ChainKernel K = chain_instance(family, P.np, F.inline_walk);
    if (user) K.name = c->u_lanes ? "user_lanes_3launches" : "user_3launches";
    if (c->obj == SMM_OBJ_DENSE && c->dense2) K.name = "iter<dense2,16>";
    if (obj_kind(c->obj) == 0 && K.tpw == 1 && !walk && !F.inline_walk) K.block = 64;
    return K;
}
ChainKernel chain_kernel_p2p(const Ctx* c) {
    const KParams& P = c->P;
    if (c->p2p_rows) return chain_instance(c->F.norm_narrow ? CF_P2P_ROWS_NARROW : CF_P2P_ROWS, P.np, false);
    return chain_instance(CF_P2P, P.np, P.Ng > XLVL_MAX || P.plan_K > XLVL_MAX);
}
void launch_chain_kernel(Ctx* c, const ChainKernel& K, size_t smem, const KParams& P, int t, const double* rec_in, double* rec_out, int flags) {
    const dim3 grid((unsigned)(((P.N + K.ct - 1) / K.ct + K.tpw - 1) / K.tpw)), block(K.block);
    void* args[] = {(void*)&P, (void*)&t, (void*)&rec_in, (void*)&rec_out, (void*)&flags};
    launch_fn(c, K.fn, grid, block, smem, c->stream, args);
// ... 9 lines not shown
    const hipFunction_t fn = base_seed ? c->ufn_noseed : c->ufn;
    if (c->u_lanes > 0)
        HIPCHK(hipModuleLaunchKernel(fn, (unsigned)n, 1, 1, (unsigned)c->u_lanes, 1, 1, 0, c->stream, args, nullptr));
    else
        HIPCHK(hipModuleLaunchKernel(fn, (unsigned)((n + 127) / 128), 1, 1, 128, 1, 1, 0, c->stream, args, nullptr));
}

enum EvalFamily { EF_BATCH, EF_SLICE, EF_LM, EF_SOBOL, EF_COUNT };
struct EvalKernel { const void* fn; int ct; };
EvalKernel eval_instance(int family, int kind) {
#define EVAL(KERN) (kind == 1 ? EvalKernel{(const void*)KERN<1, 8>, 8} : kind == 2 ? EvalKernel{(const void*)KERN<2, 16>, 16} : EvalKernel{(const void*)KERN<0, 8>, 8})
    switch (family) {
        case EF_BATCH: return EVAL(k_eval_batch);
        case EF_SLICE: return EVAL(k_eval_slice);
        case EF_LM: return EVAL(k_eval_lm);
        default: return EVAL(k_eval_sobol);
    }
#undef EVAL
}
void launch_eval_tiles(Ctx* c, int family, int n, void** args) {
    const EvalKernel K = eval_instance(family, obj_kind(c->obj));
    HIPCHK(hipLaunchKernel(K.fn, dim3((unsigned)((n + K.ct - 1) / K.ct)), dim3(WG), args, tile_smem_base(c, K.ct), c->stream));
}

void launch_eval_dev(Ctx* c, const double* params, int n, double* value, double* simM, void* status) {
    if (c->obj == SMM_OBJ_USER) {
        launch_user_kernel(c, params, n, simM, value, (int*)status);
        return;
    }
    const KParams& P = c->P;
    int8_t* st = (int8_t*)status;
    void* args[] = {(void*)&P, (void*)&params, (void*)&n, (void*)&value, (void*)&simM, (void*)&st};
    launch_eval_tiles(c, EF_BATCH, n, args);
}

void launch_chain_iter(Ctx* c, int t, int flags) {
    point_values(c, c->P, t - 1, t);
    if (c->ext_vals_out) { c->P.vals_out = c->ext_vals_out; c->P.slot8_out = nullptr; }
    const bool own_slots = c->F.xk == XK_ROWS && c->P.N == c->P.Ng && !c->ext_rec_out && !c->ext_vals_out && c->obj != SMM_OBJ_USER;
    c->P.slots17_out = own_slots ? c->slots17 : nullptr;
    c->P.nan_flags_out = own_slots ? c->nan_flags + (t & 1) : nullptr;
    if (own_slots) c->run.slots_iter = t;
    const ChainKernel K = chain_kernel(c, flags);
    const size_t smem = tile_smem(c, c->F, K.ct, K.tpw);
    const double* rin = c->ext_rec_in ? c->ext_rec_in : (const double*)c->rec[c->run.cur];
    double* rout = c->ext_rec_out ? c->ext_rec_out : c->rec[c->run.cur ^ 1];
    if (c->obj == SMM_OBJ_USER) {
        const KParams& P = c->P;
        launch_chain_kernel(c, K, smem, P, t, rin, rout, flags | F_PROPOSE_ONLY);
        launch_user_kernel(c, P.u_theta, P.N, P.u_simM, P.u_value, P.u_status);
    }
    launch_chain_kernel(c, K, smem, c->P, t, rin, rout, flags);
    if (!c->ext_rec_out) c->run.cur ^= 1;
}

constexpr size_t ROWS_OWN_MAX = (size_t)158 * 1024;
ExchInstance exch_instance(int id, int Ng) {
    const size_t rows_all = resolve_rows_bytes(XKEY_MAX, XKEY_MAX, XROWS_MAX), rows_part = resolve_rows_bytes(XKEY_PARTNER_MAX, XKEY_PARTNER_MAX, XROWS_MAX),
                 lvl = resolve_lvl_bytes(XLVL_MAX, XLVL_MAX);
    switch (id) {
        case XI_CONE_CHAINS: return {(const void*)k_cone_chains, XWG, cone_chains_lds_bytes(Ng), XG_CONE_BIG, "cone_chains", false};
        case XI_CONE_TILES: return {(const void*)k_cone_tiles, 64 * CONEB_WAVES, 0, XG_CONE_BIG, "cone_tiles", false};
        case XI_PLAN_BIG: return {(const void*)k_exch_plan_big, XWG, plan_big_lds_bytes(65535), XG_BIG, "plan_big", false};
        case XI_PLAN: return {(const void*)k_exch_plan, XWG, plan_smem(XLDS_MAX, XLDS_MAX, true), XG_LDS, "plan", false};
        case XI_LEAN: return {(const void*)k_exch_resolve_lean, XWG, LDS_CU, XG_LDS, "lean", true};
#ifdef SMM_TEST_HOOKS
        case XI_LVL_256: return {(const void*)k_exch_resolve_lvl<256>, 256, lvl, XG_LDS, "lvl", false};
        case XI_LVL_512: return {(const void*)k_exch_resolve_lvl<512>, 512, lvl, XG_LDS, "lvl", false};
        case XI_TICKETS: return {(const void*)k_exch_resolve_lds, XWG, resolve_lds_bytes(XLDS_MAX), XG_LDS, "tickets", false};
#endif
        case XI_LVL: return {(const void*)k_exch_resolve_lvl<1024>, 1024, lvl, XG_LDS, "lvl", true};
        case XI_LVL_SOA: return {(const void*)k_exch_resolve_lvl_soa<1024>, 1024, resolve_lvl_soa_bytes(XLDS_MAX, XLDS_MAX), XG_LDS, "lvl_soa", false};
        case XI_KEYS: return {(const void*)k_exch_keys, 256, 0, XG_KEYS, "keys", false};
        case XI_ROWS_PLDS: return {(const void*)k_exch_resolve_rows<true>, XWG, rows_part, XG_KEYS, "rows", false};
        case XI_ROWS: return {(const void*)k_exch_resolve_rows<false>, XWG, rows_all, XG_KEYS, "rows", false};
        case XI_KEY_PLDS: return {(const void*)k_exch_resolve_key<true>, XWG, resolve_key_bytes(XKEY_PARTNER_MAX, XKEY_PARTNER_MAX), XG_KEYS, "key", false};
        case XI_KEY: return {(const void*)k_exch_resolve_key<false>, XWG, resolve_key_bytes(XKEY_MAX, XKEY_MAX), XG_KEYS, "key", false};
        case XI_LVL_BIG: return {(const void*)k_exch_resolve_lvl_big, XWG, 0, XG_BIG, "lvl_big", false};
        case XI_ANY: return {(const void*)k_exch_resolve_any, XWG, 0, XG_BIG, "any", false};
        case XI_ROWS_WIN_OWN: return {(const void*)k_exch_resolve_rows<false, true, true>, XWG, ROWS_OWN_MAX, XG_KEYS, "rows_window_own", true};
        case XI_ROWS_WIN_PLDS: return {(const void*)k_exch_resolve_rows<true, true>, XWG, rows_part, XG_KEYS, "rows_window", true};
        case XI_ROWS_WIN: return {(const void*)k_exch_resolve_rows<false, true>, XWG, rows_all, XG_KEYS, "rows_window", true};
        case XI_APPLY: return {(const void*)k_exch_apply, 256, 0, XG_BIG, "apply", false};
        default: return {nullptr, 0, 0, XG_LDS, id == XI_TICKETS ? "tickets" : "lvl", false};
    }
}
ExchLaunch resolve_kernel(const Ctx* c, const KParams& P) {
    const bool plds = P.Ng <= XKEY_PARTNER_MAX;
    switch (c->F.xk) {
        case XK_LEAN: return {XI_LEAN, resolve_lean_bytes(P.Ng, P.plan_K, P.lean_wide != 0)};
        case XK_LVL: return {c->H.lvl_wg == 256 ? XI_LVL_256 : c->H.lvl_wg == 512 ? XI_LVL_512 : XI_LVL, resolve_lvl_bytes(P.Ng, P.plan_K)};
        case XK_LVL_SOA: return {XI_LVL_SOA, resolve_lvl_soa_bytes(P.Ng, P.plan_K)};
        case XK_TICKETS: return {XI_TICKETS, resolve_lds_bytes(P.Ng)};
        case XK_ROWS: return {plds ? XI_ROWS_PLDS : XI_ROWS, resolve_rows_bytes(P.Ng, P.plan_K, P.rows_cap)};
        case XK_KEY: return {plds ? XI_KEY_PLDS : XI_KEY, resolve_key_bytes(P.Ng, P.plan_K)};
        case XK_LVL_BIG: return {XI_LVL_BIG, 0};
        default: return {XI_ANY, 0};
    }
}
ExchLaunch resolve_rows_window_kernel(const Ctx* c) {
    const KParams& P = c->P;
    const size_t own = resolve_rows_bytes(P.Ng, P.plan_K, P.rows_cap, P.N);
    if (P.Ng > XKEY_PARTNER_MAX && P.N < P.Ng && own <= ROWS_OWN_MAX) return {XI_ROWS_WIN_OWN, own};
    return {P.Ng <= XKEY_PARTNER_MAX ? XI_ROWS_WIN_PLDS : XI_ROWS_WIN, resolve_rows_bytes(P.Ng, P.plan_K, P.rows_cap)};
}
bool resolve_stamped(const Ctx* c, bool shard) {
    const int id = resolve_kernel(c, c->P).id;
    return exch_instance(id).stamped && (shard ? id == XI_LEAN : c->P.Ng <= XLVL_MAX && !c->H.dataflow && c->H.lvl_wg == 1024);
}

void launch_resolve_p(Ctx* c, const KParams& P_in, int t, const double* gathered) {
    KParams P = P_in;
    point_values(c, P, t, t);
    const ExchLaunch L = resolve_kernel(c, P);
    if (c->F.xk != XK_ROWS && c->F.xk != XK_KEY) return launch_exch(c, L.id, dim3(1), L.smem, c->stream, P, t, gathered);
    const bool prepass = gathered || c->run.slots_iter != t;
    const double* vals = gathered ? P.xval : P.vals;
    const uint32_t *slots16 = prepass ? (const uint32_t*)P.xsrc : nullptr, *slots17 = c->slots17;
    if (prepass)
        launch_exch(c, XI_KEYS, dim3((P.Ng + 255) / 256), 0, c->stream, gathered ? gathered : (const double*)P.vals, gathered ? P.RW : 1, P.Ng, (double*)vals, (uint32_t*)P.xsrc,
                    c->F.xk == XK_ROWS ? c->slots17 : (uint32_t*)nullptr, c->nan_flags, t);
    if (c->F.xk == XK_ROWS) launch_exch(c, L.id, dim3(1), L.smem, c->stream, P, t, vals, slots16, slots17, c->nan_flags);
    else launch_exch(c, L.id, dim3(1), L.smem, c->stream, P, t, vals, (const uint32_t*)P.xsrc);
}
void launch_resolve(Ctx* c, int t, const double* gathered) { launch_resolve_p(c, c->P, t, gathered); }

size_t p2p_walk_bytes(const Ctx* c) { return (LeanLayout<LEAN_KEYS>::bytes(c->P.Ng, c->P.plan_K) + 15) & ~(size_t)15; }
void launch_chain_iter_norm_p2p(Ctx* c, int t, int flags) {
    KParams P = c->P;
    point_values(c, P, t - 1, t);
    const bool walk = (flags & F_WALK_INLINE) != 0;
    P.tile_off = walk ? (int)(p2p_walk_bytes(c) / sizeof(double)) : 0;
    const size_t smem = (size_t)P.tile_off * sizeof(double) + norm_tile_doubles(P.np) * sizeof(double);
    launch_chain_kernel(c, chain_kernel_p2p(c), smem, P, t, nullptr, nullptr, flags);
}
void launch_p2p_push(Ctx* c, int t, const double* rec_src, bool ll) {
    KParams P = c->P;
    const dim3 grid(p2p_units(P.N)), block(256);
    if (ll) hipLaunchKernelGGL((k_p2p_push<true, true>), grid, block, 0, c->stream, P, t, rec_src);
    else if (rec_src) hipLaunchKernelGGL((k_p2p_push<true, false>), grid, block, 0, c->stream, P, t, rec_src);
    else hipLaunchKernelGGL((k_p2p_push<false, false>), grid, block, 0, c->stream, P, t, (const double*)nullptr);
    if (!ll) { c->p2p_seq += 1; c->p2p_unwaited = true; }
}
void launch_p2p_wait(Ctx* c) {
    KParams P = c->P;
    P.p2p_want = (unsigned long long)p2p_units(P.N) * c->p2p_seq;
    hipLaunchKernelGGL(k_p2p_wait, dim3(1), dim3(64), 0, c->stream, P, c->run.iter);
    c->p2p_unwaited = false;
}
void launch_p2p_unpack(Ctx* c, int t) {
    hipLaunchKernelGGL(k_p2p_unpack, dim3((c->P.Ng + 255) / 256), dim3(256), 0, c->stream, c->P, t);
}
void launch_resolve_window(Ctx* c, int t) {
    const P2PLayout L = p2p_layout(c->P.Ng, c->P.RW);
    KParams P1 = c->P;
    P1.RW = 1;
    launch_resolve_p(c, P1, t, (const double*)(c->p2p_mine + L.val[t & 1]));
}
void launch_resolve_rows_window(Ctx* c, int t) {
    const ExchLaunch L = resolve_rows_window_kernel(c);
    launch_exch(c, L.id, dim3(1), L.smem, c->stream, c->P, t, (const double*)nullptr, (const uint32_t*)nullptr, (const uint32_t*)nullptr, (uint32_t*)nullptr);
}
enum PersistId { PI_GEN, PI_LOC_PCT, PI_LOC = PI_LOC_PCT + 2, PI_TILE = PI_LOC + 8, PI_COUNT = PI_TILE + 10 };
enum PersistTileVariant { PT_SHARD, PT_CHOL_PCT, PT_CHOL, PT_PCT, PT_PLAIN };
struct PersistInstance { const void* fn; unsigned block; const char* name; };
PersistInstance persist_instance(int id) {
// ... 55 lines not shown
```

### smm.jl_amd/csrc/smm_lookahead.hpp

```cpp
#pragma once
__global__ void k_pregen_rng(const KParams P, const int t0, const int W, double* __restrict__ rb) {
    const int N = P.N, np = P.np, TR = P.rb_tries;
    const int Q = (np + 1) / 2;
    const uint32_t per_iter = (uint32_t)TR * (uint32_t)Q * (uint32_t)N;
    const uint32_t i = blockIdx.x * blockDim.x + threadIdx.x;
    if (i >= per_iter) return;
    const int q = (int)(i % (uint32_t)Q);
    const uint32_t rest = i / (uint32_t)Q;
    const int r = (int)(rest % (uint32_t)TR);
    const int c = (int)(rest / (uint32_t)TR);
    const int w = (int)blockIdx.y;
    const int t = t0 + w;
    const uint32_t gc = (uint32_t)(P.offset + c);
    double* blk = rb + ((size_t)w * N + c) * P.RBW;
    if (t > 1) {
        double z0, z1 = 0.0;
        if (P.user_ntab) {
            const size_t base = (((size_t)(t - 1) * TR + r) * np) * N + c;
            z0 = P.user_ntab[base + (size_t)(2 * q) * N];
            if (2 * q + 1 < np) z1 = P.user_ntab[base + (size_t)(2 * q + 1) * N];
        } else {
            rng_prop_normal2(P.seed, gc, (uint32_t)t, (uint32_t)r, (uint32_t)q, z0, z1);
        }
        blk[1 + r * np + 2 * q] = z0;
// ... 324 lines not shown
                    uint32_t bits = need[(size_t)q * wpp + w];
                    while (bits) {
                        const uint32_t b = (uint32_t)w * 32u + (uint32_t)__builtin_ctz(bits);
                        bits &= bits - 1u;
                        atomicAdd(&lcnt[b * LS + lvq[m]], 1u);
                    }
                }
        }
        __syncthreads();
        if (P.ts && blockIdx.x == 0 && tid == 0) P.ts[(size_t)8 * 60000 + 87] = wall_clock64();
        for (int b = tid; b < nb; b += XWG) {
            uint32_t sub = 0;
            uint32_t hw[CONE_HDRW];
#pragma unroll
            for (int x = 0; x < CONE_HDRW; ++x) hw[x] = 0u;
            for (int l = 1; l <= nlev; ++l) {
                const uint32_t n = lcnt[b * LS + l];
                lcnt[b * LS + l] = sub * 64u;
                for (uint32_t x = 0; x < n; x += 64u, ++sub)
                    if (sub < (uint32_t)CONE_LEVELS) {
                        const uint32_t cnt_s = n - x < 64u ? n - x : 64u;
#pragma unroll
                        for (int y = 0; y < CONE_LEVELS / 4; ++y)
                            if ((int)(sub >> 2) == y) hw[1 + y] |= cnt_s << (8u * (sub & 3u));
                    }
            }
            hw[0] = sub <= (uint32_t)CONE_LEVELS ? sub : 0u;
            if (sub > (uint32_t)CONE_LEVELS) atomicOr(&s_bad, 1u);
#pragma unroll
            for (int x = 0; x < CONE_HDRW; ++x) o_hdr[(size_t)(b0 + b) * CONE_HDRW + x] = hw[x];
        }
        __syncthreads();
        if (P.ts && blockIdx.x == 0 && tid == 0) P.ts[(size_t)8 * 60000 + 88] = wall_clock64();
#pragma unroll
        for (int m = 0; m < MAXPP; ++m) {
            const int q = tid + m * XWG;
            if (q < K) {
                const uint32_t word = (sc8 * ci[m]) | ((sc8 * cj[m]) << 16);
                const bool gi = o_gl && rri[m] == 0, gj = o_gl && rrj[m] == 0;
                const uint32_t ti = ((uint32_t)ci[m] - (uint32_t)P.offset) / ct, tj = ((uint32_t)cj[m] - (uint32_t)P.offset) / ct;
                for (int w = 0; w < wpp; ++w) {
                    uint32_t bits = need[(size_t)q * wpp + w];
                    while (bits) {
                        uint32_t bb[4], dst[4], g1[4], g2[4];
#pragma unroll
                        for (int u = 0; u < 4; ++u) {
                            bb[u] = 0xffffffffu;
                            if (bits) { bb[u] = (uint32_t)w * 32u + (uint32_t)__builtin_ctz(bits); bits &= bits - 1u; }
                        }
#pragma unroll
                        for (int u = 0; u < 4; ++u) {
                            dst[u] = 0u; g1[u] = 0xffffffffu; g2[u] = 0xffffffffu;
                            if (bb[u] != 0xffffffffu) {
                                dst[u] = atomicAdd(&lcnt[bb[u] * LS + lvq[m]], 1u);
                                if (gi && ti != (uint32_t)b0 + bb[u]) g1[u] = atomicAdd(&gcnt[bb[u]], 1u);
                                if (gj && tj != (uint32_t)b0 + bb[u]) g2[u] = atomicAdd(&gcnt[bb[u]], 1u);
                            }
                        }
#pragma unroll
                        for (int u = 0; u < 4; ++u)
                            if (bb[u] != 0xffffffffu) {
                                if (dst[u] < (uint32_t)(CONE_LEVELS * 64)) o_cp[(size_t)(b0 + bb[u]) * (CONE_LEVELS * 64) + dst[u]] = word;
                                if (g1[u] < (uint32_t)CONE_GCAP) o_gl[(size_t)(b0 + bb[u]) * CONE_GCAP + g1[u]] = ci[m];
                                if (g2[u] < (uint32_t)CONE_GCAP) o_gl[(size_t)(b0 + bb[u]) * CONE_GCAP + g2[u]] = cj[m];
                            }
                    }
                }
            }
        }
        if (o_gl) {
            __syncthreads();
            for (int b = tid; b < nb; b += XWG) {
                const uint32_t g = gcnt[b];
                if (g > (uint32_t)CONE_GCAP) { atomicOr(&s_bad, 1u); o_hdr[(size_t)(b0 + b) * CONE_HDRW] = 0u; }
                else o_hdr[(size_t)(b0 + b) * CONE_HDRW] |= g << 16;
            }
        }
    }
    __syncthreads();
    if (P.ts && blockIdx.x == 0 && tid == 0) P.ts[(size_t)8 * 60000 + 89] = wall_clock64();
    if (tid == 0) *o_ok = s_bad ? 0u : 1u;
}
__host__ __device__ inline size_t plan_cone_bytes() { return (size_t)152 * 1024; }
```

### smm.jl_amd/csrc/smmhip.hip

```cpp
#include <hip/hip_runtime.h>
#include <hip/hip_ext.h>
#include <hip/hiprtc.h>
#include <dlfcn.h>
#include <chrono>
#include <mutex>
#include <thread>
#include <stdint.h>
#include <stdio.h>
#include <string.h>
#include <stdlib.h>
#include <math.h>
#include <algorithm>
#include <string>
#include <vector>
#include <type_traits>

#include "../../include/smmhip.h"
#include "smm_rng.hpp"

namespace {

using namespace smm;

#include "smm_params.hpp"
// ... 69 lines not shown
    int hist_lds_bins = 1 << 30;
    size_t pop_scratch = 0;
    size_t opt_scratch = 0;
    bool opt_materialise = false;
};
Hooks read_hooks() {
    Hooks H;
    auto is = [](const char* v, char ch) { return v && v[0] == ch; };
    if (const char* v = SMM_HOOK("SMMHIP_FILL")) H.fill = atoi(v);
    H.any_exchange = is(SMM_HOOK("SMMHIP_ANY_EXCHANGE"), '1');
    H.dataflow = is(SMM_HOOK("SMMHIP_DATAFLOW_EXCHANGE"), '1');
    H.big_exchange = is(SMM_HOOK("SMMHIP_BIG_EXCHANGE"), '1');
    H.key_exchange_off = is(SMM_HOOK("SMMHIP_KEY_EXCHANGE"), '0');
    H.key_walk_off = is(SMM_HOOK("SMMHIP_KEY_WALK"), '0');
    H.inline_walk_off = is(SMM_HOOK("SMMHIP_INLINE_WALK"), '0');
    H.norm_fast_off = is(SMM_HOOK("SMMHIP_NORM_FAST"), '0');
    if (const char* v = SMM_HOOK("SMMHIP_NORM_NARROW")) H.norm_narrow = v[0] == '0' ? 0 : v[0] == '1' ? 1 : -1;
    if (const char* v = SMM_HOOK("SMMHIP_TPW")) H.tpw = v[0] == '1' ? 1 : v[0] == '2' ? 2 : 0;
    H.dense_keys_off = is(SMM_HOOK("SMMHIP_DENSE_KEYS"), '0');
    H.no_cone = is(SMM_HOOK("SMMHIP_NO_CONE"), '1');
    H.persist_off = is(SMM_HOOK("SMMHIP_PERSIST"), '0');
    H.persist_loc_off = is(SMM_HOOK("SMMHIP_PERSIST_LOC"), '0');
    H.persist_tile_off = is(SMM_HOOK("SMMHIP_PERSIST_TILE"), '0');
    H.cone_big_off = is(SMM_HOOK("SMMHIP_CONE_BIG"), '0');
    H.plan_ahead_off = is(SMM_HOOK("SMMHIP_PLAN_AHEAD"), '0');
    if (const char* v = SMM_HOOK("SMMHIP_PLAN_CAP")) H.plan_cap = atoi(v);
    if (const char* v = SMM_HOOK("SMMHIP_LVL_WG")) H.lvl_wg = atoi(v);
    if (const char* v = SMM_HOOK("SMMHIP_SCOUT_AFTER")) H.scout_after = atoi(v);
    if (const char* v = SMM_HOOK("SMMHIP_SCOUT_GL")) H.scout_gl = atoi(v) == 8 ? 8 : 16;
    if (const char* v = SMM_HOOK("SMMHIP_A2A_CAP")) H.a2a_cap = std::max(1, atoi(v));
    if (const char* v = SMM_HOOK("SMMHIP_PR_RING")) { const int k = atoi(v); if (k == 2 || k == 4) H.pr_ring_k = k; }
    if (const char* v = SMM_HOOK("SMMHIP_PR_SLOW_TILE")) H.pr_slow_tile = atoi(v);
    if (const char* v = SMM_HOOK("SMMHIP_PR_SLOW_US")) H.pr_slow_ticks = 100 * atoi(v);
    H.pr_slow_read = is(SMM_HOOK("SMMHIP_PR_SLOW_READ"), '1');
    H.rows_win_check = SMM_HOOK("SMMHIP_ROWS_WIN_CHECK") != nullptr;
    if (const char* v = SMM_HOOK("SMMHIP_STATS_SCRATCH")) H.stats_scratch = (size_t)strtoull(v, nullptr, 10);
    if (const char* v = SMM_HOOK("SMMHIP_STATS_MODE_BINS")) H.stats_mode_bins = std::min(STATS_MODE_BINS, std::max(1, atoi(v)));
    if (const char* v = SMM_HOOK("SMMHIP_GROUP_WIDE_MIN")) H.group_wide_min = std::min((long long)STATS_LDS_N + 1, std::max(1ll, atoll(v)));
    if (const char* v = SMM_HOOK("SMMHIP_HIST_LDS_BINS")) H.hist_lds_bins = std::max(1, atoi(v));
    if (const char* v = SMM_HOOK("SMMHIP_POP_SCRATCH")) H.pop_scratch = (size_t)strtoull(v, nullptr, 10);
    if (const char* v = SMM_HOOK("SMMHIP_OPT_SCRATCH")) H.opt_scratch = (size_t)strtoull(v, nullptr, 10);
    H.opt_materialise = is(SMM_HOOK("SMMHIP_OPT_MATERIALISE"), '1');
    return H;
}
enum ExchKernel { XK_LEAN, XK_LVL, XK_LVL_SOA, XK_TICKETS, XK_ROWS, XK_KEY, XK_LVL_BIG, XK_ANY };
enum PlanKind { PLAN_NONE, PLAN_LDS, PLAN_BIG };
enum PersistKind { PERSIST_NONE, PERSIST_GEN, PERSIST_LOC, PERSIST_TILE };
struct Forms {
    PlanKind plan = PLAN_NONE;
    ExchKernel xk = XK_ANY;
    int rows_cap = 0;
    bool lean_plan = false;
    bool lean_wide = false;
    bool plan_ahead = false;
    int win_cap = 0;
    int plan_cap = 0;
    int ct = 8;
    bool norm_fast = false;
    bool norm_narrow = false;
    int tpw = 1;
    int tile_off = 0;
    bool inline_walk = false;
    bool gen_lean = false;
    bool gen_keys = false;
    bool dense_keys = false;
    bool cone = false;
    bool cone_big = false;
    bool walk_slots = false;
    int cone_tiles = 0, cone_ct = 0;
    bool cone_gather = false;
    PersistKind persist = PERSIST_NONE;
    bool persist_wide = false;
    bool persist_sh = false;
    bool persist_sh_big = false;
    bool persist_user = false;
    int max_tiles = 0;
    bool defer_resolve = false;
};

struct DeviceFacts { int n_cus = 256; int per_cu = -1; };
struct ChainKernel { const void* fn; const char* name; unsigned block; int ct, tpw; };
struct PersistKernel { const void* fn; hipFunction_t mfn; dim3 grid, block; size_t smem; std::string name; };
enum ExchId { XI_CONE_CHAINS, XI_CONE_TILES, XI_PLAN_BIG, XI_PLAN, XI_LEAN, XI_LVL_256, XI_LVL_512, XI_LVL, XI_LVL_SOA, XI_TICKETS, XI_KEYS, XI_ROWS_PLDS,
              XI_ROWS, XI_KEY_PLDS, XI_KEY, XI_LVL_BIG, XI_ANY, XI_ROWS_WIN_OWN, XI_ROWS_WIN_PLDS, XI_ROWS_WIN, XI_APPLY, XI_COUNT };
enum ExchGroup { XG_BIG, XG_KEYS, XG_LDS, XG_CONE_BIG };
struct ExchInstance { const void* fn; unsigned block; size_t cap; ExchGroup group; const char* name; bool stamped; };
struct ExchLaunch { int id; size_t smem; };
struct LevelTables {
    uint32_t *lv_pairs = nullptr, *lv_off = nullptr, *lv_rows = nullptr, *lv_rowinfo = nullptr, *cone_ok = nullptr, *cone_hdr = nullptr, *cone_pairs = nullptr;
    double* lv_mi = nullptr; uint16_t* cone_gather = nullptr;
};
struct Run {
    int iter = 0;
    int cur = 0;
    int slots_iter = -1;
    bool pending = false;
    bool prev_open = false;
    bool unresolved = false;
    bool exch_done = false;
};

struct Ctx {
    KParams P{};
    Hooks H;
    Forms F;
    DeviceFacts dev;
    bool has_chol = false, dense2 = false, has_ntab = false, has_utab = false;
    int obj = 0, device = 0, exchange_from = 2;
    hipStream_t stream = nullptr;
    hipEvent_t ev0 = nullptr, ev1 = nullptr;
    std::vector<void*> allocs;
    std::string err;
    int u_lanes = 0;
    int n_objp = 0;
    hipModule_t umod = nullptr;
    hipFunction_t ufn = nullptr;
    hipFunction_t ufn_noseed = nullptr;
    bool u_rng = false;
    hipModule_t pmod = nullptr;
    hipFunction_t pfn = nullptr;
    int u_nsums = 1;
    std::vector<std::pair<int32_t, hipModule_t>> tmods;
    int pop_kind = 0, pop_M = 0;
    double pop_spread = 0.0;

    Run run;
    bool rec_external = false;
    bool pending_ext = false;
    bool a2a_open = false;
    bool p2p_current = false;
    bool p2p_unwaited = false;
    int failed = 0;
    bool failed_told = false;
    double* rec[2] = {nullptr, nullptr};
    double* vals_buf[2] = {nullptr, nullptr};
    uint2* slot8_buf[2] = {nullptr, nullptr};
    bool deep_plan = false;
    bool nan_values = false;
    const double* ext_rec_in = nullptr;
    double* ext_rec_out = nullptr;
    double* ext_vals_out = nullptr;

    double* win_rb = nullptr;
    unsigned long long* win_plan = nullptr;
    double* win_plan_mi = nullptr;
    LevelTables win;
    uint32_t *win_lv_pairs_p = nullptr, *win_lv_offp = nullptr, *slots17 = nullptr, *nan_flags = nullptr;
    uint32_t* big_scratch = nullptr;
    int rng_t0 = 0, rng_w = 0;
    int plan_t0 = 0, plan_w = 0;
    uint32_t* cb_scratch = nullptr;
    std::vector<uint32_t> cone_big_ok;
    struct PlanSet : LevelTables {
        uint32_t* ok_host = nullptr;
        hipEvent_t done = nullptr;
        int t0 = 0, w = 0;
    } ps[2];
    int ps_act = 0;
    hipStream_t pstream = nullptr;
    hipEvent_t ev_free = nullptr;

    int32_t *a2a_send_idx = nullptr, *a2a_send_cnt = nullptr, *a2a_rowidx = nullptr;
    int a2a_cap = 0, a2a_G = 0;

    unsigned char* p2p_mine = nullptr;
    void* p2p_opened[P2P_MAXG] = {};
    unsigned p2p_attached = 0;
    unsigned long long p2p_seq = 0;
    bool p2p_inline = false;
    bool p2p_rows = false;
    bool p2p_mode_inline = false;
    int p2p_ranks_here = 1;

    unsigned char* prw = nullptr;
    size_t prw_off = 0;
    bool persist_proven = false;
    int persist_strikes = 0;
    int persist_on = 1;
    bool persist_broken = false;
    uint32_t pr_epoch = 0;
    int persist_launches = 0, persist_repairs = 0;
    int pregen_seen_launches = 0;
    bool in_repair = false;
    bool snap_valid = false;
    Run snap;
    double *snap_cs = nullptr, *snap_rec = nullptr, *snap_vals[2] = {nullptr, nullptr}, *hist_fill = nullptr;
    uint2* snap_slot8[2] = {nullptr, nullptr};
    unsigned long long* snap_xres = nullptr;

    void* st_scr = nullptr;
    size_t st_scr_bytes = 0;
    void* red_res = nullptr;
    size_t red_res_bytes = 0;

    smm_timing_t timing{};
    bool pending_timing = false;
    int profiling = 0;
    hipEvent_t kev0 = nullptr, kev1 = nullptr;
    std::vector<char> pev_exch;
    std::vector<hipEvent_t> pev;
    int pev_iters = 0;
};

#define HIPCHK(call)                                                                                  \
    do {                                                                                              \
        hipError_t e_ = (call);                                                                       \
        if (e_ != hipSuccess) {                                                                       \
            char b_[512];                                                                             \
            snprintf(b_, sizeof b_, "%s failed: %s (%s:%d)", #call, hipGetErrorString(e_), __FILE__, __LINE__); \
            throw std::string(b_);                                                                    \
        }                                                                                             \
    } while (0)

template <class T>
T* dalloc(Ctx* c, size_t n) {
    void* p = nullptr;
    HIPCHK(hipMalloc(&p, (n ? n : 1) * sizeof(T)));
    c->allocs.push_back(p);
    if (c->H.fill >= 0) HIPCHK(hipMemset(p, c->H.fill, (n ? n : 1) * sizeof(T)));
    return (T*)p;
}
template <class T>
T* dupload(Ctx* c, const T* h, size_t n) {
    T* d = dalloc<T>(c, n);
    if (h && n) HIPCHK(hipMemcpy(d, h, n * sizeof(T), hipMemcpyHostToDevice));
    return d;
}

void launch_fn(Ctx* c, const void* fn, dim3 grid, dim3 block, size_t smem, hipStream_t st, void** args, bool stamped = true) {
    if (stamped && c->kev0 && st == c->stream) HIPCHK(hipExtLaunchKernel(fn, grid, block, args, smem, st, c->kev0, c->kev1, 0));
    else HIPCHK(hipLaunchKernel(fn, grid, block, args, smem, st));
}

bool is_sim(int obj) { return obj == SMM_OBJ_NORM || obj == SMM_OBJ_NORM_FAILBOX; }
int obj_kind(int obj) { return is_sim(obj) ? 1 : obj == SMM_OBJ_DENSE ? 2 : 0; }
void point_values(const Ctx* c, KParams& P, int t_read, int t_write) {
    P.vals = c->vals_buf[t_read & 1]; P.vals_out = c->vals_buf[t_write & 1];
    P.slot8 = c->slot8_buf[t_read & 1]; P.slot8_out = c->slot8_buf[t_write & 1];
}

// ... 205 lines not shown
        if (s->iter > c->P.T) return SMM_ERR_INVALID_ARG;
        if (s->iter > 0 && !h) return fail(c, SMM_ERR_INVALID_ARG, "history of iterations 0..iter-1 required");
        if (!s->sigma || !s->accept_rate || !s->n_noex || !s->n_acc_noex || !s->best_val || !s->best_id || !s->la_value ||
            !s->la_prob || !s->la_status || !s->la_params || !s->la_sim_moments)
            return fail(c, SMM_ERR_INVALID_ARG, "smm_set_state needs every field of smm_state_t");
        if (s->iter > 0 && (!h->value || !h->prob || !h->curr_val || !h->best_val || !h->params || !h->sim_moments ||
                            !h->best_id || !h->exchanged || !h->accepted || !h->status))
            return fail(c, SMM_ERR_INVALID_ARG, "smm_set_state needs every field of smm_history_t");
        if (const int rc = estimate_enter(c)) return rc;
        KParams& P = c->P;
        const size_t N = P.N, RW = P.RW, HW = P.HW, np = P.np, nm = P.nm;
        std::vector<double> cs(N * CSW), rec(N * RW, 0.0);
        HIPCHK(hipMemcpy(cs.data(), P.cs, cs.size() * 8, hipMemcpyDeviceToHost));
        bool nan_seen = false;
        for (size_t i = 0; i < N; ++i) {
            double* b = cs.data() + i * CSW;
            double* r = rec.data() + i * RW;
            b[CS_SIGMA] = s->sigma[i]; b[CS_RATE] = s->accept_rate[i];
            b[CS_NNOEX] = (double)s->n_noex[i]; b[CS_NACC] = (double)s->n_acc_noex[i];
            b[CS_LACC] = 0.0; b[CS_WASX] = 0.0;
            b[CS_BEST] = s->best_val[i]; b[CS_BESTID] = (double)s->best_id[i];
            b[CS_BESTP] = s->best_val[i]; b[CS_BESTPID] = (double)s->best_id[i];
            r[0] = s->la_value[i]; r[1] = s->la_prob[i]; r[2] = (double)s->la_status[i];
            if (s->la_value[i] != s->la_value[i]) nan_seen = true;
            for (size_t k = 0; k < np; ++k) r[3 + k] = s->la_params[k * N + i];
            for (size_t k = 0; k < nm; ++k) r[3 + np + k] = s->la_sim_moments[k * N + i];
        }
        c->nan_values = nan_seen;
        HIPCHK(hipMemcpy(P.cs, cs.data(), cs.size() * 8, hipMemcpyHostToDevice));
        HIPCHK(hipMemcpy(c->rec[c->run.cur], rec.data(), rec.size() * 8, hipMemcpyHostToDevice));
        std::vector<double> row(N * HW, 0.0);
        for (int t = 0; t < s->iter; ++t) {
            const size_t o = (size_t)t * N;
            for (size_t i = 0; i < N; ++i) {
                double* hr = row.data() + i * HW;
                history_head(hr, h->value[o + i], h->prob[o + i], h->curr_val[o + i], h->best_val[o + i], (double)h->best_id[o + i],
                             (double)h->exchanged[o + i], (double)h->accepted[o + i], (double)h->status[o + i]);
                for (size_t k = 0; k < np; ++k) hr[H_PARAMS + k] = h->params[((size_t)t * np + k) * N + i];
                for (size_t k = 0; k < nm; ++k) hr[H_PARAMS + np + k] = h->sim_moments[((size_t)t * nm + k) * N + i];
            }
            HIPCHK(hipMemcpy(P.hrec + (size_t)t * N * HW, row.data(), row.size() * 8, hipMemcpyHostToDevice));
        }
        c->run.iter = s->iter;
        if (c->failed) {
            const unsigned long long e = ERR_NONE;
            HIPCHK(hipMemcpy(P.err, &e, 8, hipMemcpyHostToDevice));
            c->failed = 0; c->failed_told = false;
        }
        c->rec_external = false; c->pending_ext = false; c->run.unresolved = false;
        c->run.pending = false;
        c->run.prev_open = false;
        c->a2a_open = false;
        c->p2p_current = false;
        c->run.exch_done = false;
        c->run.slots_iter = -1;
        if (P.walk_flags) HIPCHK(hipMemset(P.walk_flags, 0, 16));
        return SMM_OK;
    });
}

int smm_get_timing(void* ctx, smm_timing_t* out) {
    Ctx* c = (Ctx*)ctx;
    if (!c || !out) return SMM_ERR_INVALID_ARG;
    *out = c->timing;
    return SMM_OK;
}

int smm_set_persistent(void* ctx, int32_t on) {
    Ctx* c = (Ctx*)ctx;
    if (!c) return SMM_ERR_INVALID_ARG;
    c->persist_on = on ? 1 : 0;
    return SMM_OK;
}

int smm_get_persistent(void* ctx, int32_t* available, int32_t* launches, int32_t* repairs) {
    Ctx* c = (Ctx*)ctx;
    if (!c) return SMM_ERR_INVALID_ARG;
    if (available) *available = (c->F.persist != PERSIST_NONE && c->persist_on && !c->persist_broken) ? 1 : 0;
    if (launches) *launches = c->persist_launches;
    if (repairs) *repairs = c->persist_repairs;
    return SMM_OK;
}

int smm_set_profiling(void* ctx, int32_t on) {
    Ctx* c = (Ctx*)ctx;
    if (!c) return SMM_ERR_INVALID_ARG;
    c->profiling = on < 0 ? 0 : (on > 2 ? 2 : on);
    return SMM_OK;
}

int smm_debug_ts(void* ctx, unsigned long long* out, int n_wg) {
    Ctx* c = (Ctx*)ctx;
    if (!c || !c->P.ts) return SMM_ERR_INVALID_ARG;
    if (n_wg == -2) {
        if (hipMemcpy(out, c->P.ts + PL_LATE_BASE, (size_t)PL_LATE_N * 8, hipMemcpyDeviceToHost) != hipSuccess) return SMM_ERR_HIP;
        return SMM_OK;
    }
    if (n_wg < 0) {
        if (hipMemcpy(out, c->P.ts + (size_t)8 * 60000, 8 * 100, hipMemcpyDeviceToHost) != hipSuccess) return SMM_ERR_HIP;
        return SMM_OK;
    }
    if (hipMemcpy(out, c->P.ts, (size_t)n_wg * 8 * 8, hipMemcpyDeviceToHost) != hipSuccess) return SMM_ERR_HIP;
    return SMM_OK;
}
int smm_debug_ts_waves(void* ctx, unsigned long long* out, int n_wg) {
    Ctx* c = (Ctx*)ctx;
    if (!c || !c->P.ts || n_wg < 0 || n_wg > PL_TSW_TILES) return SMM_ERR_INVALID_ARG;
    const size_t words = (size_t)n_wg * (NORM_WG / 64) * PL_TSW;
    if (hipMemcpy(out, c->P.ts + PL_TSW_BASE, words * 8, hipMemcpyDeviceToHost) != hipSuccess) return SMM_ERR_HIP;
    return SMM_OK;
}

#ifdef SMM_TEST_HOOKS
int smm_debug_plan_window(void* ctx, int t, double* ms_out, int* window_out) {
    return api_call(ctx, ms_out != nullptr, [&](Ctx* c) -> int {
        HIPCHK(hipSetDevice(c->device));
        hipEvent_t e0, e1;
        HIPCHK(hipEventCreate(&e0)); HIPCHK(hipEventCreate(&e1));
        c->plan_w = 0;
        HIPCHK(hipEventRecord(e0, c->stream));
        ensure_windows(c, t, false);
        HIPCHK(hipEventRecord(e1, c->stream));
        HIPCHK(hipEventSynchronize(e1));
        float ms = 0.f;
        HIPCHK(hipEventElapsedTime(&ms, e0, e1));
        *ms_out = ms;
        if (window_out) *window_out = c->plan_w;
        (void)hipEventDestroy(e0); (void)hipEventDestroy(e1);
        return SMM_OK;
    });
}
int smm_debug_cone(void* ctx, int w, int tile, uint32_t* hdr, uint32_t* pairs, uint16_t* gather, int32_t* info) {
    Ctx* c = (Ctx*)ctx;
    if (!c || !c->P.cone_hdr) return SMM_ERR_INVALID_ARG;
    const KParams& P = c->P;
    if (hipStreamSynchronize(c->stream) != hipSuccess) return SMM_ERR_HIP;
    if (hipMemcpy(hdr, P.cone_hdr + ((size_t)w * P.cone_tiles + tile) * CONE_HDRW, CONE_HDRW * 4, hipMemcpyDeviceToHost) != hipSuccess) return SMM_ERR_HIP;
    if (hipMemcpy(pairs, P.cone_pairs + ((size_t)w * P.cone_tiles + tile) * (CONE_LEVELS * 64), CONE_LEVELS * 64 * 4, hipMemcpyDeviceToHost) != hipSuccess) return SMM_ERR_HIP;
    if (P.cone_gather && hipMemcpy(gather, P.cone_gather + ((size_t)w * P.cone_tiles + tile) * CONE_GCAP, CONE_GCAP * 2, hipMemcpyDeviceToHost) != hipSuccess) return SMM_ERR_HIP;
    uint32_t ok = 0;
    if (hipMemcpy(&ok, P.cone_ok + w, 4, hipMemcpyDeviceToHost) != hipSuccess) return SMM_ERR_HIP;
    info[0] = c->plan_t0; info[1] = c->plan_w; info[2] = (int32_t)ok; info[3] = P.cone_ct;
    return SMM_OK;
}
#endif

int smm_get_Z(void* ctx, double* Z) {
    return api_call(ctx, Z != nullptr, [&](Ctx* c) -> int {
        HIPCHK(hipSetDevice(c->device));
        for (int k = 0; k < c->P.nm; ++k)
            HIPCHK(hipMemcpy(Z + (size_t)k * c->P.ns, c->P.Z + (size_t)k * c->P.zstride, (size_t)c->P.ns * sizeof(double),
                             hipMemcpyDeviceToHost));
        return SMM_OK;
    });
}

}
```

### smm.jl_amd/host.py

```python
import time as _time
from builtins import range as _builtins_range
from collections import OrderedDict

import numpy as np

from . import _abi as A
from .backend import BGPOpts, Problem, Tables, hip_context


class DeviceObjective:
    def __init__(self, name, objective_id, ns=10000, needs_square=False):
        self.name, self.objective_id, self.ns, self.needs_square = name, objective_id, ns, needs_square

    def __call__(self, ev, **opts):
        return evaluateObjective(ev._mprob, ev) if getattr(ev, "_mprob", None) is not None else _no_mprob()

    def __repr__(self):
        return "<device objective %s>" % self.name


def _no_mprob():
    raise ValueError("a device objective needs an Eval built from an MProb (Eval(mprob, p))")


# ... 947 lines not shown
    elif method == "lm":
        res = lm_results(algo.m, algo._ctx.opt_lm(starts, **simplex))
    else:
        res = opt_results(algo.m, algo._ctx.opt_slices(starts, npoints, tol, update, maxiter))
    names = ps2s_names(algo.m)
    for s, (r, (label, j)) in enumerate(zip(res, who)):
        r["start"] = {per: label, "p": OrderedDict((k, float(starts[i, s])) for i, k in enumerate(names)), "value": float(bv[j])}
    return sorted(res, key=lambda r: r["best"]["value"])


class ABCPMCResult:

    def __init__(self, names, raw):
        self.names, self.raw = list(names), raw
        self.n_kept, self.generations, self.status, self.ess, self.evaluated = (raw[f] for f in ("n_kept", "generations", "status", "ess", "evaluated"))
        self.eps = raw["eps"][:self.generations + 1]
        self.p_acc = raw["p_acc"][:self.generations + 1]

    def mean(self):
        return OrderedDict((k, float(v)) for k, v in zip(self.names, self.raw["mean"]))

    def cov(self):
        return np.array(self.raw["cov"])

    def quantile(self):
        return OrderedDict((k, [float(v) for v in self.raw["quantile"][:, i]]) for i, k in enumerate(self.names))

    def draws(self):
        n = self.n_kept
        return np.array(self.raw["theta"][:, :n]), np.array(self.raw["weight"][:n])


def abc_pmc(algo, n_particles, keep=0.5, max_gen=20, p_acc_min=0.05, scale=2.0, ridge=0.0, probs=(0.025, 0.5, 0.975)):
    A = int(keep) if keep >= 2 else int(np.floor(keep * n_particles))
    return ABCPMCResult(ps2s_names(algo.m), algo._ctx.abc_pmc(n_particles, A, max_gen, p_acc_min, scale, ridge, probs))


class SobolResult:

    def __init__(self, params, moments, raw):
        self.params, self.outputs, self.raw = list(params), ["value"] + list(moments), raw
        self.n_complete, self.n_invalid, self.evaluated = (raw[f] for f in ("n_complete", "n_invalid", "evaluated"))

    def _table(self, a):
        return OrderedDict((o, OrderedDict((k, float(a[f, i])) for i, k in enumerate(self.params))) for f, o in enumerate(self.outputs))

    def first(self):
        return self._table(self.raw["first"])

    def total(self):
        return self._table(self.raw["total"])

    def interaction(self):
        return self._table(self.raw["total"] - self.raw["first"])

    def se(self):
        return {"first": self._table(self.raw["se_first"]), "total": self._table(self.raw["se_total"])}

    def ranking(self, output="value"):
        t = self.raw["total"][self.outputs.index(output)]
        return [self.params[i] for i in sorted(range(len(self.params)), key=lambda i: (np.isnan(t[i]), -t[i] if not np.isnan(t[i]) else 0.0))]

    def unidentified(self, tol=1e-3):
        t = self.raw["total"][1:]
        return [k for i, k in enumerate(self.params) if all(not (v > tol) for v in t[:, i])]


def global_sensitivity(algo, n_base=4096, box=None):
    return _sobol_result(algo.m, algo._ctx, n_base, box)


def _sobol_result(m, ctx, n_base, box):
    names = ps2s_names(m)
    lo = hi = None
    if box is not None:
        unknown = [k for k in box if k not in names]
        if unknown:
            raise KeyError("global_sensitivity: %s are no sampled parameters" % unknown)
        bounds = [box.get(k, (m.params_to_sample[k]["lb"], m.params_to_sample[k]["ub"])) for k in names]
        lo, hi = [float(b[0]) for b in bounds], [float(b[1]) for b in bounds]
    return SobolResult(names, ms_names(m), ctx.sens_sobol(n_base, lo, hi))


def set_proposal(algo, L):
    algo._ctx.set_proposal(L)


def adapt_proposal(algo, window=None, accepted_only=True, min_draws=None, normalize=True, ridge=1e-8):
    t0, t1 = (0, algo.i) if window is None else window
    st = algo._ctx.adapt_proposal(t0, t1, accepted_only, min_draws, normalize, ridge)
    algo._invalidate()
    return st


def save(algo, filename):
    h, s = algo._ctx.history(0, algo.i), algo._ctx.state()
    d = {"i": algo.i}
    if algo._ctx.proposal_layout is not None:
        d["chol_L"] = algo._ctx.proposal()
    d.update({"h_" + f: getattr(h, f) for f in A.HistoryBuffers.FIELDS})
    d.update({"s_" + f: getattr(s, f) for f in A.StateBuffers.FIELDS})
    np.savez(filename if filename.endswith(".npz") else filename + ".npz", **d)


def readMalgo(algo, filename):
    z = np.load(filename if filename.endswith(".npz") else filename + ".npz")
    i = int(z["i"])
    hb = A.HistoryBuffers(i, algo._ctx.N, algo._ctx.np, algo._ctx.nm)
    sb = A.StateBuffers(algo._ctx.N, algo._ctx.np, algo._ctx.nm)
    for f in A.HistoryBuffers.FIELDS:
        getattr(hb, f)[...] = z["h_" + f]
    for f in A.StateBuffers.FIELDS:
        getattr(sb, f)[...] = z["s_" + f]
    sb.iter = i
    algo._ctx.set_state(sb, hb)
    if "chol_L" in z.files:
        algo._ctx.set_proposal(z["chol_L"])
    algo.i = i
    algo._invalidate()
    return algo


def restart(algo, extra_iter):
    new_maxiter = int(algo.opts["maxiter"]) + int(extra_iter)
    tb = algo._tables
    if tb is not None and tb.covers_iterations() is not None and tb.covers_iterations() < new_maxiter:
        raise ValueError("restart: the injected randomness tables cover %d iterations, the extended run needs %d — "
                         "build the MAlgoBGP with tables for the whole run, or without tables" % (tb.covers_iterations(), new_maxiter))
    h, s = algo._ctx.history(0, algo.i), algo._ctx.state()
    algo.opts["maxiter"] = new_maxiter
    bo = algo._bopts
    bo.maxiter = new_maxiter
    if algo._ctx.proposal_layout is not None:
        bo.chol_L = algo._ctx.proposal()
    algo._ctx.close()
    algo._ctx = hip_context(algo._prob, bo, tb)
    s.iter = algo.i
    algo._ctx.set_state(s, h)
    algo._invalidate()
    return run(algo)


def snorm_impl(opts, niter=200, npar=2):
    pb = OrderedDict()
    pb["p1"] = [0.2, -3, 3]
    pb["p2"] = [-0.2, -20, 20]
    moms = {"name": ["mu1", "mu2"], "value": [-1.0, 10.0], "weight": [1.0, 1.0]}
    if npar > 2:
        rng = np.random.default_rng(12)

        def map_range(a1, a2, b1, b2, x):
            return b1 + (x - a1) * (b2 - b1) / (a2 - a1)
        spaces = np.concatenate([rng.random(2), [4.0 ** -4], (np.linspace(0.25, 0.45, npar - 1) ** -4.0)[::-1]])
        for j in range(3, npar + 1):
            sp = float(spaces[j - 1])
            pb["p%d" % j] = [map_range(0, 1, -sp, sp, rng.random()), -sp, sp]
            y = map_range(0, 1, -sp, sp, rng.random())
            moms["name"].append("mu%d" % j); moms["value"].append(y); moms["weight"].append(y)
    mprob = MProb()
    addSampledParam(mprob, pb)
    addMoment(mprob, moms)
    addEvalFunc(mprob, objfunc_norm)
    MA = MAlgoBGP(mprob, opts)
    run(MA)
    return MA

# ... 7 lines not shown
```

Baseline: 360.7 million.

## Build exchange plans on a side stream beside the persistent chain kernel

Adds a low-register, LDS-sized background plan kernel (k_exch_plan_bg) that computes the next exchange-plan window on a separate non-blocking stream. Two plan sets are double-buffered, so the main stream only waits on an event instead of launching the plan kernel in-stream. The persistent chain kernel gets a VGPR cap so both kernels can be co-resident, and its wave priorities are raised so the simulation still wins scheduling. The VGPR cap risks spills, and the path is active only when several layout and occupancy conditions hold.

```diff
diff --git a/include/smmhip.h b/include/smmhip.h
--- a/include/smmhip.h
+++ b/include/smmhip.h
@@ -488,6 +488,7 @@
 int  smm_set_profiling(void* ctx, int32_t on);
 int  smm_set_persistent(void* ctx, int32_t on);
 int  smm_get_persistent(void* ctx, int32_t* available, int32_t* launches, int32_t* repairs);
+int  smm_get_plan_beside(void* ctx, int32_t* beside, int32_t* windows_beside, int32_t* windows_instream);
 int  smm_describe(void* ctx, char* out, int32_t cap);
 int  smm_get_Z(void* ctx, double* Z);
 
diff --git a/smm.jl_amd/_abi.py b/smm.jl_amd/_abi.py
--- a/smm.jl_amd/_abi.py
+++ b/smm.jl_amd/_abi.py
@@ -320,6 +320,7 @@
     ("smm_set_profiling", C.c_int, [C.c_void_p, C.c_int32]),
     ("smm_set_persistent", C.c_int, [C.c_void_p, C.c_int32]),
     ("smm_get_persistent", C.c_int, [C.c_void_p, C.POINTER(C.c_int32), C.POINTER(C.c_int32), C.POINTER(C.c_int32)]),
+    ("smm_get_plan_beside", C.c_int, [C.c_void_p, C.POINTER(C.c_int32), C.POINTER(C.c_int32), C.POINTER(C.c_int32)]),
     ("smm_describe", C.c_int, [C.c_void_p, C.c_char_p, C.c_int32]),
 ]
 
diff --git a/smm.jl_amd/backend.py b/smm.jl_amd/backend.py
--- a/smm.jl_amd/backend.py
+++ b/smm.jl_amd/backend.py
@@ -635,6 +635,11 @@
         self._check(self._fn("get_persistent")(self._ctx, C.byref(a), C.byref(l), C.byref(r)))
         return bool(a.value), int(l.value), int(r.value)
 
+    def plan_beside_info(self):
+        b, wb, wi = C.c_int32(0), C.c_int32(0), C.c_int32(0)
+        self._check(self._fn("get_plan_beside")(self._ctx, C.byref(b), C.byref(wb), C.byref(wi)))
+        return bool(b.value), int(wb.value), int(wi.value)
+
     def Z(self):
         z = np.empty((self.nm, self.problem.ns))
         self._check(self._fn("get_Z")(self._ctx, A.dptr(z)))
diff --git a/smm.jl_amd/csrc/smm_chain_persist_loc.hpp b/smm.jl_amd/csrc/smm_chain_persist_loc.hpp
--- a/smm.jl_amd/csrc/smm_chain_persist_loc.hpp
+++ b/smm.jl_amd/csrc/smm_chain_persist_loc.hpp
@@ -2,6 +2,7 @@
 constexpr int PL_LOCN = NORM_CT + CONE_GCAP + 2;
 constexpr uint32_t PL_PBASE = ((16u * PL_LOCN + 127u) & ~127u);
 constexpr int PL_HASH = 1024;
+constexpr int PL_VGPR_HALF = 60;
 constexpr size_t PL_TSW_BASE = (size_t)8 * 8192;
 constexpr int PL_TSW_TILES = 2048, PL_TSW = 8;
 constexpr size_t PL_LATE_BASE = PL_TSW_BASE + (size_t)PL_TSW_TILES * (NORM_WG / 64) * PL_TSW;
@@ -113,7 +114,7 @@
 }
 
 template <int NP, bool WIDE, bool SH, bool PCT = false>
-__global__ __launch_bounds__(NORM_WG, 4) void k_chain_persist_loc(const PersistArgs A) {
+__global__ __launch_bounds__(NORM_WG, 4) __attribute__((amdgpu_num_vgpr(PL_VGPR_HALF))) void k_chain_persist_loc(const PersistArgs A) {
     static_assert(!PCT || (WIDE && !SH), "thresholds by chain: the wide walk of a single shard");
     static_assert(NP == 1 || NP == 2, "one moment per half of the workgroup");
     extern __shared__ __attribute__((aligned(16))) unsigned char lds[];
@@ -139,6 +140,7 @@
     auto exch_on = [&](const int tx) { return exch_any && tx >= A.exch_from; };
 
     if (error_before(*(const volatile unsigned long long*)A.err, t0)) return;
+    __builtin_amdgcn_s_setprio(1);
 
     if (tid < 64) {
         const int cl = lane >> 2, r = lane & 3, c = tile * CT + cl;
@@ -424,14 +426,14 @@
             unsigned long long tw0 = 0, tw1 = 0, tw2 = 0;
             if (A.ts) tw0 = wall_clock64();
             if (simw) {
-                __builtin_amdgcn_s_setprio(1);
+                __builtin_amdgcn_s_setprio(2);
                 if (nfull == PR_ZR - 1) persist_simulate<NP, true>(z, nfull, extra, Y.s_theta, Y.s_part, h, wih, A.ts != nullptr, tw1);
                 else persist_simulate<NP, false>(z, nfull, extra, Y.s_theta, Y.s_part, h, wih, A.ts != nullptr, tw1);
                 if (A.ts) tw2 = wall_clock64();
                 __builtin_amdgcn_fence(__ATOMIC_RELEASE, "workgroup");
                 const int lane3 = (int)__builtin_amdgcn_mbcnt_hi(~0u, __builtin_amdgcn_mbcnt_lo(~0u, 0u));
                 if (lane3 == 0) __hip_atomic_fetch_add(Y.s_arrived, 1u, __ATOMIC_RELAXED, __HIP_MEMORY_SCOPE_WORKGROUP);
-                __builtin_amdgcn_s_setprio(0);
+                __builtin_amdgcn_s_setprio(1);
             }
             const int lane = (int)__builtin_amdgcn_mbcnt_hi(~0u, __builtin_amdgcn_mbcnt_lo(~0u, 0u));
             const bool lists = t < t1 && exch_on(t);
@@ -650,13 +652,13 @@
                     st[CS_WASX] = (double)src;
                 }
             }
-            __builtin_amdgcn_s_setprio(1);
+            __builtin_amdgcn_s_setprio(2);
             if (nfull0 == PR_ZR - 1) persist_simulate<NP, true>(z0, nfull0, extra0, Y.s_theta, Y.s_part, 0, 0, A.ts != nullptr, tw1);
             else persist_simulate<NP, false>(z0, nfull0, extra0, Y.s_theta, Y.s_part, 0, 0, A.ts != nullptr, tw1);
             if (A.ts) tw2 = wall_clock64();
             __builtin_amdgcn_fence(__ATOMIC_RELEASE, "workgroup");
             if (lane_a == 0) __hip_atomic_fetch_add(Y.s_arrived, 1u, __ATOMIC_RELAXED, __HIP_MEMORY_SCOPE_WORKGROUP);
-            __builtin_amdgcn_s_setprio(0);
+            __builtin_amdgcn_s_setprio(1);
         }
         {
             const unsigned want = (unsigned)(8 * NP) * (unsigned)rel;
diff --git a/smm.jl_amd/csrc/smm_create_host.hpp b/smm.jl_amd/csrc/smm_create_host.hpp
--- a/smm.jl_amd/csrc/smm_create_host.hpp
+++ b/smm.jl_amd/csrc/smm_create_host.hpp
@@ -263,6 +263,18 @@
     if (F.cone_tiles) { P.cone_tiles = F.cone_tiles; P.cone_ct = F.cone_ct; }
 }
 
+constexpr size_t LDS_GRANULE = 1280;
+bool plan_beside_resident(int np) {
+    auto up = [](size_t b) { return (b + LDS_GRANULE - 1) / LDS_GRANULE * LDS_GRANULE; };
+    return up(persist_loc_smem_bytes(np)) + up(PBG_LDS + PBG_LDS_STATIC) <= LDS_CU && PBG_LDS > LDS_HALF && 4 * 2 * PL_VGPR_HALF + 2 * PBG_VGPR_HALF <= 512;
+}
+void choose_plan_beside(Ctx* c) {
+    const Forms& F = c->F;
+    const KParams& P = c->P;
+    c->plan_beside = F.plan == PLAN_LDS && F.persist == PERSIST_LOC && !F.persist_sh && P.N == P.Ng && F.cone_tiles > 0 && F.cone_gather && F.plan_cap >= 2 &&
+                     !c->H.plan_ahead_off && plan_bg_fits(P.Ng, P.plan_K) && plan_beside_resident(P.np);
+}
+
 void alloc_windows(Ctx* c) {
     KParams& P = c->P;
     const Forms& F = c->F;
@@ -292,6 +304,20 @@
         HIPCHK(hipMemset(P.walk_flags, 0, 16));
     }
     if (F.cone_big || F.persist_sh_big) c->cb_scratch = dalloc<uint32_t>(c, W * cone_big_scratch_words(P.Ng, P.plan_K));
+    if (c->plan_beside) {
+        HIPCHK(hipStreamCreateWithFlags(&c->pstream, hipStreamNonBlocking));
+        HIPCHK(hipEventCreateWithFlags(&c->ev_free, hipEventDisableTiming));
+        static_cast<LevelTables&>(c->ps[0]) = c->win;
+        c->ps[0].plan = c->win_plan; c->ps[0].plan_mi = c->win_plan_mi; c->ps[0].lv_pairs_p = c->win_lv_pairs_p; c->ps[0].lv_offp = c->win_lv_offp;
+        alloc_level_tables(c, c->ps[1], false, (size_t)F.cone_tiles, F.cone_gather);
+        c->ps[1].plan = dalloc<unsigned long long>(c, W * K);
+        c->ps[1].plan_mi = dalloc<double>(c, W * K);
+        if (F.lean_plan) {
+            c->ps[1].lv_pairs_p = dalloc<uint32_t>(c, W * P.plan_Kp + 512);
+            c->ps[1].lv_offp = dalloc<uint32_t>(c, W * LV_OFFP);
+        }
+        for (Ctx::PlanSet& S : c->ps) HIPCHK(hipEventCreateWithFlags(&S.done, hipEventDisableTiming));
+    }
     if (F.plan_ahead) {
         HIPCHK(hipStreamCreateWithFlags(&c->pstream, hipStreamNonBlocking));
         HIPCHK(hipEventCreateWithFlags(&c->ev_free, hipEventDisableTiming));
@@ -418,6 +444,7 @@
         if (const char* why = create_facts(c, prob, opts, tab)) throw std::string(why);
         upload_inputs(c, prob, opts, tab);
         choose_forms(c, prob->objective_id);
+        choose_plan_beside(c);
         alloc_windows(c);
         init_state(c, opts);
         if (c->F.persist != PERSIST_NONE) alloc_persist(c);
diff --git a/smm.jl_amd/csrc/smm_launch_host.hpp b/smm.jl_amd/csrc/smm_launch_host.hpp
--- a/smm.jl_amd/csrc/smm_launch_host.hpp
+++ b/smm.jl_amd/csrc/smm_launch_host.hpp
@@ -34,6 +34,18 @@
     const int W = std::min(c->F.plan_cap, Pw.T - t + 1);
     launch_plan_big(c, Pw, t, W, S, c->pstream, true);
     HIPCHK(hipMemcpyAsync(S.ok_host, S.cone_ok, (size_t)W * 4, hipMemcpyDeviceToHost, c->pstream));
+    HIPCHK(hipEventRecord(S.done, c->pstream));
+    S.t0 = t; S.w = W;
+}
+
+void plan_beside_into(Ctx* c, int k, int t) {
+    Ctx::PlanSet& S = c->ps[k];
+    KParams Pw = c->P;
+    HIPCHK(hipEventRecord(c->ev_free, c->stream));
+    HIPCHK(hipStreamWaitEvent(c->pstream, c->ev_free, 0));
+    point_tables(Pw, S);
+    const int W = std::min(c->F.plan_cap, Pw.T - t + 1);
+    launch_exch(c, XI_PLAN_BG, dim3(W), PBG_LDS, c->pstream, Pw, t, S.plan, S.plan_mi, S.lv_pairs, S.lv_mi, S.lv_off, S.lv_pairs_p, S.lv_offp);
     HIPCHK(hipEventRecord(S.done, c->pstream));
     S.t0 = t; S.w = W;
 }
@@ -82,7 +94,30 @@
         }
         point_tables(P, c->win);
     }
-    if (c->F.plan == PLAN_LDS && P.Ng > 1 && !(t >= c->plan_t0 && t < c->plan_t0 + c->plan_w)) {
+    if (c->F.plan == PLAN_LDS && c->plan_beside && P.Ng > 1 && !(t >= c->plan_t0 && t < c->plan_t0 + c->plan_w)) {
+        const int nx = c->ps_act ^ 1;
+        Ctx::PlanSet& A = c->ps[nx];
+        if (A.w > 0 && (A.t0 == t || (A.t0 == t - 1 && A.w >= 2))) {
+            HIPCHK(hipStreamWaitEvent(c->stream, A.done, 0));
+            c->ps_act = nx;
+            ++c->windows_beside;
+        } else {
+            Ctx::PlanSet& S = c->ps[c->ps_act];
+            KParams Pw = P;
+            point_tables(Pw, S);
+            const int W = std::min(c->F.plan_cap, P.T - t + 1);
+            launch_exch(c, XI_PLAN, dim3(W), plan_smem(P.Ng, P.plan_K, true), c->stream, Pw, t, S.plan, S.plan_mi, S.lv_pairs, S.lv_mi, S.lv_off, S.lv_pairs_p, S.lv_offp);
+            S.t0 = t; S.w = W;
+            ++c->windows_instream;
+        }
+        Ctx::PlanSet& S = c->ps[c->ps_act];
+        c->plan_t0 = S.t0; c->plan_w = S.w;
+        P.plan = S.plan; P.plan_mi = S.plan_mi; P.plan_t0 = S.t0;
+        point_tables(P, S);
+        P.lv_pairs_p = S.lv_pairs_p; P.lv_offp = S.lv_offp;
+        c->ps[c->ps_act ^ 1].w = 0;
+        if (S.t0 + S.w <= P.T) plan_beside_into(c, c->ps_act ^ 1, S.t0 + S.w - (S.w >= 2 && c->F.plan_cap >= 2 ? 1 : 0));
+    } else if (c->F.plan == PLAN_LDS && P.Ng > 1 && !(t >= c->plan_t0 && t < c->plan_t0 + c->plan_w)) {
         const int W = std::min(c->F.plan_cap, P.T - t + 1);
         launch_exch(c, XI_PLAN, dim3(W), plan_smem(P.Ng, P.plan_K, c->F.cone || c->F.persist != PERSIST_NONE), c->stream, P, t, c->win_plan, c->win_plan_mi,
                     c->win.lv_pairs, c->win.lv_mi, c->win.lv_off, c->win_lv_pairs_p, c->win_lv_offp);
@@ -258,6 +293,7 @@
         case XI_ROWS_WIN_PLDS: return {(const void*)k_exch_resolve_rows<true, true>, XWG, rows_part, XG_KEYS, "rows_window", true};
         case XI_ROWS_WIN: return {(const void*)k_exch_resolve_rows<false, true>, XWG, rows_all, XG_KEYS, "rows_window", true};
         case XI_APPLY: return {(const void*)k_exch_apply, 256, 0, XG_BIG, "apply", false};
+        case XI_PLAN_BG: return {(const void*)k_exch_plan_bg, PBG_WG, PBG_LDS, XG_LDS, "plan_bg", false};
         default: return {nullptr, 0, 0, XG_LDS, id == XI_TICKETS ? "tickets" : "lvl", false};
     }
 }
diff --git a/smm.jl_amd/csrc/smm_lookahead.hpp b/smm.jl_amd/csrc/smm_lookahead.hpp
--- a/smm.jl_amd/csrc/smm_lookahead.hpp
+++ b/smm.jl_amd/csrc/smm_lookahead.hpp
@@ -430,3 +430,302 @@
     if (tid == 0) *o_ok = s_bad ? 0u : 1u;
 }
 __host__ __device__ inline size_t plan_cone_bytes() { return (size_t)152 * 1024; }
+
+constexpr int PBG_WG = 256;
+constexpr int PBG_VGPR_HALF = 16;
+constexpr size_t PBG_LDS = (size_t)82 * 1024;
+constexpr size_t PBG_LDS_STATIC = 256;
+constexpr size_t PBG_HDR = 512;
+__host__ __device__ inline size_t plan_bg_pairs(const int K) { return ((size_t)K + 7) & ~(size_t)7; }
+__host__ __device__ inline size_t plan_bg_state_bytes(const int K) { return PBG_HDR + 11 * plan_bg_pairs(K); }
+__host__ __device__ inline bool plan_bg_fits(const int Ng, const int K) {
+    if (K < 1 || K > XLDS_MAX || Ng > XLDS_MAX) return false;
+    const size_t st = plan_bg_state_bytes(K), mx = (size_t)(Ng > K ? Ng : K) + 2;
+    const size_t a = (size_t)(Ng + 2) * 4 + (size_t)K * 4, b = plan_bg_pairs(K) * 2 + mx * 4, c = (size_t)K * 4 + (size_t)32 * (LV_MAXLEV + 1) * 4 + 32 * 4;
+    return st + a <= PBG_LDS && st + b <= PBG_LDS && st + c <= PBG_LDS;
+}
+__device__ inline void plan_bg_scan(uint32_t* a, const int n, uint32_t* wsum, const int tid) {
+    const int lane = tid & 63, wave = tid >> 6;
+    const int per = (n + PBG_WG - 1) / PBG_WG, c0 = tid * per;
+    uint32_t sum = 0;
+    for (int u = 0; u < per; ++u) sum += c0 + u < n ? a[c0 + u] : 0u;
+    uint32_t incl = sum;
+#pragma unroll
+    for (int off = 1; off < 64; off <<= 1) {
+        const uint32_t o = __shfl_up(incl, off, 64);
+        if (lane >= off) incl += o;
+    }
+    if (lane == 63) wsum[wave] = incl;
+    __syncthreads();
+    uint32_t run = incl - sum;
+    for (int w = 0; w < wave; ++w) run += wsum[w];
+    for (int u = 0; u < per; ++u)
+        if (c0 + u < n) { const uint32_t v = a[c0 + u]; a[c0 + u] = run; run += v; }
+    __syncthreads();
+}
+__global__ __launch_bounds__(PBG_WG) __attribute__((amdgpu_num_vgpr(PBG_VGPR_HALF))) void k_exch_plan_bg(
+    const KParams P, const int t0, unsigned long long* __restrict__ plan, double* __restrict__ plan_mi, uint32_t* __restrict__ lv_pairs,
+    double* __restrict__ lv_mi, uint32_t* __restrict__ lv_off, uint32_t* __restrict__ lv_pairs_p, uint32_t* __restrict__ lv_offp) {
+    extern __shared__ __attribute__((aligned(16))) unsigned char xsm[];
+    constexpr uint16_t NONE = 0xffffu;
+    const int tid = threadIdx.x;
+    const int t = t0 + blockIdx.x;
+    const int Ng = P.Ng, K = P.plan_K;
+    const size_t Kp = plan_bg_pairs(K);
+    uint32_t* hdr = (uint32_t*)xsm;
+    uint32_t *s_lst = hdr, *s_pst = hdr + 34, *wsum = hdr + 68, *s_nlev = hdr + 76, *s_bad = hdr + 77;
+    uint16_t* pi = (uint16_t*)(xsm + PBG_HDR);
+    uint16_t *pj = pi + Kp, *prei = pj + Kp, *prej = prei + Kp, *lvl = prej + Kp;
+    uint8_t* flg = (uint8_t*)(lvl + Kp);
+    unsigned char* tmp = xsm + plan_bg_state_bytes(K);
+    uint32_t* cnt = (uint32_t*)tmp;
+    uint16_t* ep = (uint16_t*)(cnt + Ng + 2);
+    unsigned long long* out = plan + (size_t)blockIdx.x * K;
+    double* out_mi = plan_mi + (size_t)blockIdx.x * K;
+    auto stamp = [&](const int k) { if (P.ts && blockIdx.x == 0 && tid == 0) P.ts[(size_t)8 * 60000 + 90 + k] = wall_clock64(); };
+
+    stamp(0);
+    if (tid == 0) { *s_nlev = 0u; *s_bad = 0u; }
+    for (int c = tid; c < Ng; c += PBG_WG) cnt[c] = 0;
+    if (P.pairtab) {
+        for (int q = tid; q < K; q += PBG_WG) {
+            pi[q] = (uint16_t)P.pairtab[((size_t)(t - 1) * K + q) * 2];
+            pj[q] = (uint16_t)P.pairtab[((size_t)(t - 1) * K + q) * 2 + 1];
+        }
+    } else {
+        PairPerm pp;
+        pp.init(P.seed, (uint32_t)t, (uint64_t)Ng * (uint64_t)(Ng - 1) / 2);
+        for (int q = tid; q < K; q += PBG_WG) {
+            int32_t i, j;
+            pair_unrank(pp.eval((uint64_t)q), i, j);
+            pi[q] = (uint16_t)i;
+            pj[q] = (uint16_t)j;
+        }
+    }
+    __syncthreads();
+    stamp(1);
+    for (int q = tid; q < K; q += PBG_WG) {
+        atomicAdd(&cnt[pi[q]], 1u);
+        atomicAdd(&cnt[pj[q]], 1u);
+    }
+    __syncthreads();
+    plan_bg_scan(cnt, Ng, wsum, tid);
+    for (int q = tid; q < K; q += PBG_WG) {
+        ep[atomicAdd(&cnt[pi[q]], 1u)] = (uint16_t)q;
+        ep[atomicAdd(&cnt[pj[q]], 1u)] = (uint16_t)q;
+    }
+    __syncthreads();
+    for (int q = tid; q < K; q += PBG_WG) {
+        const uint32_t i = pi[q], j = pj[q];
+        uint32_t b = i ? cnt[i - 1] : 0u, e = cnt[i], ri = 0, rj = 0;
+        for (uint32_t x = b; x < e; ++x) ri += ((uint32_t)ep[x] < (uint32_t)q) ? 1u : 0u;
+        b = j ? cnt[j - 1] : 0u; e = cnt[j];
+        for (uint32_t x = b; x < e; ++x) rj += ((uint32_t)ep[x] < (uint32_t)q) ? 1u : 0u;
+        out[q] = (unsigned long long)i | ((unsigned long long)j << 16) | ((unsigned long long)ri << 32) | ((unsigned long long)rj << 48);
+        out_mi[q] = P.min_improve_g[i];
+        prei[q] = (uint16_t)ri; prej[q] = (uint16_t)rj;
+    }
+    __syncthreads();
+    stamp(2);
+    for (int q = tid; q < K; q += PBG_WG) {
+        const uint32_t i = pi[q], j = pj[q];
+        ep[(i ? cnt[i - 1] : 0u) + prei[q]] = (uint16_t)q;
+        ep[(j ? cnt[j - 1] : 0u) + prej[q]] = (uint16_t)q;
+    }
+    __syncthreads();
+    for (int q = tid; q < K; q += PBG_WG) {
+        const uint32_t i = pi[q], j = pj[q], ri = prei[q], rj = prej[q];
+        const uint32_t bi = i ? cnt[i - 1] : 0u, bj = j ? cnt[j - 1] : 0u;
+        prei[q] = ri ? ep[bi + ri - 1] : NONE;
+        prej[q] = rj ? ep[bj + rj - 1] : NONE;
+        flg[q] = (uint8_t)((bi + ri + 1u == cnt[i] ? 1u : 0u) | (bj + rj + 1u == cnt[j] ? 2u : 0u));
+    }
+    __syncthreads();
+    uint16_t* lvl_b = (uint16_t*)tmp;
+    uint32_t* lhist = (uint32_t*)(lvl_b + Kp);
+    const int nh = (Ng > K ? Ng : K) + 2;
+    for (int q = tid; q < K; q += PBG_WG) { lvl[q] = 0; lvl_b[q] = 0; }
+    __syncthreads();
+    {
+        const uint16_t* cur = lvl;
+        uint16_t* nxt = lvl_b;
+        int changed = 1;
+        while (changed) {
+            int mine = 0;
+            for (int q = tid; q < K; q += PBG_WG) {
+                const uint32_t p1 = prei[q], p2 = prej[q];
+                const uint32_t a = p1 != NONE ? cur[p1] : 0u, b = p2 != NONE ? cur[p2] : 0u;
+                const bool known = (p1 == NONE || a) && (p2 == NONE || b);
+                const uint16_t nl = known ? (uint16_t)(1u + (a > b ? a : b)) : (uint16_t)0;
+                if (nl != cur[q]) mine = 1;
+                nxt[q] = nl;
+            }
+            changed = __syncthreads_or(mine);
+            const uint16_t* x = cur; cur = nxt; nxt = (uint16_t*)x;
+        }
+    }
+    stamp(3);
+    for (int c = tid; c < nh; c += PBG_WG) lhist[c] = 0;
+    __syncthreads();
+    {
+        uint32_t mx = 0;
+        for (int q = tid; q < K; q += PBG_WG) { const uint32_t l = lvl[q]; atomicAdd(&lhist[l], 1u); mx = l > mx ? l : mx; }
+        atomicMax(s_nlev, mx);
+    }
+    __syncthreads();
+    const int nlev = (int)*s_nlev;
+    plan_bg_scan(lhist, nlev + 1, wsum, tid);
+    uint32_t* o_off = lv_off + (size_t)blockIdx.x * (K + 2);
+    for (int l = tid; l < nlev; l += PBG_WG) o_off[l] = (l + 2 <= nlev) ? lhist[l + 2] : (uint32_t)K;
+    if (tid == 0) o_off[K + 1] = (uint32_t)nlev;
+    const bool lean = lv_pairs_p != nullptr && nlev <= LV_MAXLEV;
+    uint32_t* o_pp = lv_pairs_p ? lv_pairs_p + (size_t)blockIdx.x * P.plan_Kp : nullptr;
+    if (lv_offp && tid == 0) {
+        uint32_t* o = lv_offp + (size_t)blockIdx.x * LV_OFFP;
+        o[33] = (uint32_t)nlev; o[34] = lean ? 1u : 0u;
+        if (lean) {
+            uint32_t acc = 0;
+            for (int c = 1; c <= nlev; ++c) {
+                s_lst[c] = lhist[c]; s_pst[c] = acc; o[c - 1] = acc;
+                acc += ((c + 1 <= nlev ? lhist[c + 1] : (uint32_t)K) - lhist[c] + 63u) & ~63u;
+            }
+            s_pst[nlev + 1] = acc; o[nlev] = acc;
+        }
+    }
+    __syncthreads();
+    const uint32_t sc8 = (uint32_t)P.lean_unit;
+    if (lean) {
+        const uint32_t Ng4 = lean_Ng4(Ng);
+        const uint32_t dummy = P.lean_wide ? LeanLayout<LEAN_WIDE>::dummy_word(sc8, Ng4) : LeanLayout<LEAN_KEYS>::dummy_word(sc8, Ng4);
+        for (uint32_t q = tid; q < s_pst[nlev + 1]; q += PBG_WG) o_pp[q] = dummy;
+    }
+    __syncthreads();
+    uint32_t* o_pairs = lv_pairs + (size_t)blockIdx.x * K;
+    double* o_mi = lv_mi + (size_t)blockIdx.x * K;
+    for (int q = tid; q < K; q += PBG_WG) {
+        const uint32_t lv = lvl[q];
+        const uint32_t pos = atomicAdd(&lhist[lv], 1u);
+        const uint32_t i = pi[q], j = pj[q];
+        o_pairs[pos] = i | (j << 16);
+        o_mi[pos] = P.min_improve_g[i];
+        if (lean) o_pp[s_pst[lv] + (pos - s_lst[lv])] = (sc8 * i) | ((sc8 * j) << 16);
+    }
+    stamp(4);
+    if (P.cone_ok == nullptr) return;
+    const int tiles = P.cone_tiles;
+    uint32_t* o_ok = (uint32_t*)P.cone_ok + blockIdx.x;
+    if (!lean) {
+        if (tid == 0) *o_ok = 0u;
+        return;
+    }
+    const int LS = nlev + 1;
+    int wpp = (int)((PBG_LDS - plan_bg_state_bytes(K)) / ((size_t)K * 4 + (size_t)32 * LS * 4 + 32 * 4));
+    if (wpp > (tiles + 31) / 32) wpp = (tiles + 31) / 32;
+    if (wpp < 1) { if (tid == 0) *o_ok = 0u; return; }
+    uint32_t* need = (uint32_t*)tmp;
+    uint32_t* lcnt = need + (size_t)K * wpp;
+    uint32_t* gcnt = lcnt + (size_t)32 * wpp * LS;
+    uint16_t* o_gl = P.cone_gather ? P.cone_gather + (size_t)blockIdx.x * tiles * CONE_GCAP : nullptr;
+    uint32_t* o_hdr = (uint32_t*)P.cone_hdr + (size_t)blockIdx.x * tiles * CONE_HDRW;
+    uint32_t* o_cp = (uint32_t*)P.cone_pairs + (size_t)blockIdx.x * tiles * (CONE_LEVELS * 64);
+    const uint32_t ct = (uint32_t)P.cone_ct;
+    for (int b0 = 0; b0 < tiles; b0 += 32 * wpp) {
+        const int nb = min(32 * wpp, tiles - b0);
+        __syncthreads();
+        for (int x = tid; x < K * wpp + 32 * wpp * LS + 32 * wpp; x += PBG_WG) need[x] = 0u;
+        __syncthreads();
+        for (int q = tid; q < K; q += PBG_WG) {
+            const uint32_t f = flg[q];
+            if (f & 1u) {
+                const uint32_t b = ((uint32_t)pi[q] - (uint32_t)P.offset) / ct - (uint32_t)b0;
+                if (b < (uint32_t)nb) atomicOr(&need[(size_t)q * wpp + (b >> 5)], 1u << (b & 31u));
+            }
+            if (f & 2u) {
+                const uint32_t b = ((uint32_t)pj[q] - (uint32_t)P.offset) / ct - (uint32_t)b0;
+                if (b < (uint32_t)nb) atomicOr(&need[(size_t)q * wpp + (b >> 5)], 1u << (b & 31u));
+            }
+        }
+        stamp(5);
+        __syncthreads();
+        for (int l = nlev; l >= 2; --l) {
+            for (int q = tid; q < K; q += PBG_WG)
+                if (lvl[q] == l) {
+                    const uint32_t p1 = prei[q], p2 = prej[q];
+                    for (int w = 0; w < wpp; ++w) {
+                        const uint32_t v = need[(size_t)q * wpp + w];
+                        if (v) {
+                            if (p1 != NONE) atomicOr(&need[(size_t)p1 * wpp + w], v);
+                            if (p2 != NONE) atomicOr(&need[(size_t)p2 * wpp + w], v);
+                        }
+                    }
+                }
+            __syncthreads();
+        }
+        stamp(6);
+        for (int q = tid; q < K; q += PBG_WG) {
+            const uint32_t lv = lvl[q];
+            for (int w = 0; w < wpp; ++w) {
+                uint32_t bits = need[(size_t)q * wpp + w];
+                while (bits) {
+                    const uint32_t b = (uint32_t)w * 32u + (uint32_t)__builtin_ctz(bits);
+                    bits &= bits - 1u;
+                    atomicAdd(&lcnt[b * LS + lv], 1u);
+                }
+            }
+        }
+        __syncthreads();
+        stamp(7);
+        for (int b = tid; b < nb; b += PBG_WG) {
+            uint32_t sub = 0;
+            uint32_t* oh = o_hdr + (size_t)(b0 + b) * CONE_HDRW;
+            for (int x = 0; x < CONE_HDRW; ++x) oh[x] = 0u;
+            for (int l = 1; l <= nlev; ++l) {
+                const uint32_t n = lcnt[b * LS + l];
+                lcnt[b * LS + l] = sub * 64u;
+                for (uint32_t x = 0; x < n; x += 64u, ++sub)
+                    if (sub < (uint32_t)CONE_LEVELS) {
+                        const uint32_t cnt_s = n - x < 64u ? n - x : 64u;
+                        oh[1 + (sub >> 2)] |= cnt_s << (8u * (sub & 3u));
+                    }
+            }
+            oh[0] = sub <= (uint32_t)CONE_LEVELS ? sub : 0u;
+            if (sub > (uint32_t)CONE_LEVELS) atomicOr(s_bad, 1u);
+        }
+        __syncthreads();
+        stamp(8);
+        for (int q = tid; q < K; q += PBG_WG) {
+            const uint32_t i = pi[q], j = pj[q], lv = lvl[q];
+            const uint32_t word = (sc8 * i) | ((sc8 * j) << 16);
+            const bool gi = o_gl && prei[q] == NONE, gj = o_gl && prej[q] == NONE;
+            const uint32_t ti = (i - (uint32_t)P.offset) / ct, tj = (j - (uint32_t)P.offset) / ct;
+            for (int w = 0; w < wpp; ++w) {
+                uint32_t bits = need[(size_t)q * wpp + w];
+                while (bits) {
+                    const uint32_t bb = (uint32_t)w * 32u + (uint32_t)__builtin_ctz(bits);
+                    bits &= bits - 1u;
+                    const uint32_t dst = atomicAdd(&lcnt[bb * LS + lv], 1u);
+                    if (dst < (uint32_t)(CONE_LEVELS * 64)) o_cp[(size_t)(b0 + bb) * (CONE_LEVELS * 64) + dst] = word;
+                    if (gi && ti != (uint32_t)b0 + bb) {
+                        const uint32_t g = atomicAdd(&gcnt[bb], 1u);
+                        if (g < (uint32_t)CONE_GCAP) o_gl[(size_t)(b0 + bb) * CONE_GCAP + g] = (uint16_t)i;
+                    }
+                    if (gj && tj != (uint32_t)b0 + bb) {
+                        const uint32_t g = atomicAdd(&gcnt[bb], 1u);
+                        if (g < (uint32_t)CONE_GCAP) o_gl[(size_t)(b0 + bb) * CONE_GCAP + g] = (uint16_t)j;
+                    }
+                }
+            }
+        }
+        if (o_gl) {
+            __syncthreads();
+            for (int b = tid; b < nb; b += PBG_WG) {
+                const uint32_t g = gcnt[b];
+                if (g > (uint32_t)CONE_GCAP) { atomicOr(s_bad, 1u); o_hdr[(size_t)(b0 + b) * CONE_HDRW] = 0u; }
+                else o_hdr[(size_t)(b0 + b) * CONE_HDRW] |= g << 16;
+            }
+        }
+    }
+    __syncthreads();
+    stamp(9);
+    if (tid == 0) *o_ok = *s_bad ? 0u : 1u;
+}
diff --git a/smm.jl_amd/csrc/smmhip.hip b/smm.jl_amd/csrc/smmhip.hip
--- a/smm.jl_amd/csrc/smmhip.hip
+++ b/smm.jl_amd/csrc/smmhip.hip
@@ -175,7 +175,7 @@
 struct ChainKernel { const void* fn; const char* name; unsigned block; int ct, tpw; };
 struct PersistKernel { const void* fn; hipFunction_t mfn; dim3 grid, block; size_t smem; std::string name; };
 enum ExchId { XI_CONE_CHAINS, XI_CONE_TILES, XI_PLAN_BIG, XI_PLAN, XI_LEAN, XI_LVL_256, XI_LVL_512, XI_LVL, XI_LVL_SOA, XI_TICKETS, XI_KEYS, XI_ROWS_PLDS,
-              XI_ROWS, XI_KEY_PLDS, XI_KEY, XI_LVL_BIG, XI_ANY, XI_ROWS_WIN_OWN, XI_ROWS_WIN_PLDS, XI_ROWS_WIN, XI_APPLY, XI_COUNT };
+              XI_ROWS, XI_KEY_PLDS, XI_KEY, XI_LVL_BIG, XI_ANY, XI_ROWS_WIN_OWN, XI_ROWS_WIN_PLDS, XI_ROWS_WIN, XI_APPLY, XI_PLAN_BG, XI_COUNT };
 enum ExchGroup { XG_BIG, XG_KEYS, XG_LDS, XG_CONE_BIG };
 struct ExchInstance { const void* fn; unsigned block; size_t cap; ExchGroup group; const char* name; bool stamped; };
 struct ExchLaunch { int id; size_t smem; };
@@ -248,7 +248,12 @@
         uint32_t* ok_host = nullptr;
         hipEvent_t done = nullptr;
         int t0 = 0, w = 0;
+        unsigned long long* plan = nullptr;
+        double* plan_mi = nullptr;
+        uint32_t *lv_pairs_p = nullptr, *lv_offp = nullptr;
     } ps[2];
+    bool plan_beside = false;
+    int windows_beside = 0, windows_instream = 0;
     int ps_act = 0;
     hipStream_t pstream = nullptr;
     hipEvent_t ev_free = nullptr;
@@ -620,6 +625,15 @@
     return SMM_OK;
 }
 
+int smm_get_plan_beside(void* ctx, int32_t* beside, int32_t* windows_beside, int32_t* windows_instream) {
+    return api_call(ctx, true, [&](Ctx* c) -> int {
+        if (beside) *beside = c->plan_beside ? 1 : 0;
+        if (windows_beside) *windows_beside = c->windows_beside;
+        if (windows_instream) *windows_instream = c->windows_instream;
+        return SMM_OK;
+    });
+}
+
 int smm_set_profiling(void* ctx, int32_t on) {
     Ctx* c = (Ctx*)ctx;
     if (!c) return SMM_ERR_INVALID_ARG;
@@ -650,6 +664,74 @@
 }
 
 #ifdef SMM_TEST_HOOKS
+int smm_debug_plan_beside_budget(int np, int Ng, int K, long long* out) {
+    if (!out || np < 1 || np > 2) return SMM_ERR_INVALID_ARG;
+    out[0] = (long long)persist_loc_smem_bytes(np); out[1] = (long long)PBG_LDS; out[2] = (long long)LDS_CU; out[3] = (long long)LDS_GRANULE;
+    int n = 0;
+    while (plan_bg_fits(n + 1, n + 1)) ++n;
+    out[4] = n; out[5] = plan_bg_fits(Ng, K) && plan_beside_resident(np) ? 1 : 0; out[6] = (long long)PBG_LDS_STATIC;
+    return SMM_OK;
+}
+static int debug_plan_sets(Ctx* c) {
+    if (c->plan_beside) return c->P.cone_tiles;
+    if (c->F.plan != PLAN_LDS || !c->F.lean_plan || c->F.plan_ahead) return 0;
+    const int tiles = (c->P.N + NORM_CT - 1) / NORM_CT;
+    if (!c->ps[0].plan) {
+        const size_t W = (size_t)c->F.plan_cap, K = (size_t)c->P.plan_K;
+        for (Ctx::PlanSet& S : c->ps) {
+            alloc_level_tables(c, S, false, (size_t)tiles, true);
+            S.plan = dalloc<unsigned long long>(c, W * K); S.plan_mi = dalloc<double>(c, W * K);
+            S.lv_pairs_p = dalloc<uint32_t>(c, W * c->P.plan_Kp + 512); S.lv_offp = dalloc<uint32_t>(c, W * LV_OFFP);
+        }
+    }
+    return tiles;
+}
+int smm_debug_plan_tables(void* ctx, int which, int w, int32_t* info, unsigned long long* plan, uint32_t* lv_pairs, uint32_t* lv_off, uint32_t* offp, uint32_t* pairs_p,
+                          uint32_t* hdr, uint32_t* cpairs, uint16_t* gather) {
+    return api_call(ctx, info != nullptr, [&](Ctx* c) -> int {
+        HIPCHK(hipSetDevice(c->device));
+        const size_t tiles = (size_t)debug_plan_sets(c);
+        if (!tiles) return SMM_ERR_INVALID_ARG;
+        HIPCHK(hipStreamSynchronize(c->stream));
+        if (c->pstream) HIPCHK(hipStreamSynchronize(c->pstream));
+        const Ctx::PlanSet& S = c->ps[which < 0 ? c->ps_act : (which & 1)];
+        const KParams& P = c->P;
+        const size_t K = (size_t)P.plan_K;
+        uint32_t ok = 0, nlev = 0;
+        HIPCHK(hipMemcpy(&ok, S.cone_ok + w, 4, hipMemcpyDeviceToHost));
+        HIPCHK(hipMemcpy(&nlev, S.lv_off + (size_t)w * (K + 2) + K + 1, 4, hipMemcpyDeviceToHost));
+        info[0] = S.t0; info[1] = S.w; info[2] = (int32_t)nlev; info[3] = (int32_t)ok; info[4] = (int32_t)K; info[5] = (int32_t)tiles; info[6] = P.plan_Kp; info[7] = S.lv_pairs_p ? 1 : 0;
+        if (plan) HIPCHK(hipMemcpy(plan, S.plan + (size_t)w * K, K * 8, hipMemcpyDeviceToHost));
+        if (lv_pairs) HIPCHK(hipMemcpy(lv_pairs, S.lv_pairs + (size_t)w * K, K * 4, hipMemcpyDeviceToHost));
+        if (lv_off) HIPCHK(hipMemcpy(lv_off, S.lv_off + (size_t)w * (K + 2), (K + 2) * 4, hipMemcpyDeviceToHost));
+        if (offp && S.lv_offp) HIPCHK(hipMemcpy(offp, S.lv_offp + (size_t)w * LV_OFFP, LV_OFFP * 4, hipMemcpyDeviceToHost));
+        if (pairs_p && S.lv_pairs_p) HIPCHK(hipMemcpy(pairs_p, S.lv_pairs_p + (size_t)w * P.plan_Kp, (size_t)P.plan_Kp * 4, hipMemcpyDeviceToHost));
+        if (hdr) HIPCHK(hipMemcpy(hdr, S.cone_hdr + (size_t)w * tiles * CONE_HDRW, tiles * CONE_HDRW * 4, hipMemcpyDeviceToHost));
+        if (cpairs) HIPCHK(hipMemcpy(cpairs, S.cone_pairs + (size_t)w * tiles * (CONE_LEVELS * 64), tiles * CONE_LEVELS * 64 * 4, hipMemcpyDeviceToHost));
+        if (gather && S.cone_gather) HIPCHK(hipMemcpy(gather, S.cone_gather + (size_t)w * tiles * CONE_GCAP, tiles * CONE_GCAP * 2, hipMemcpyDeviceToHost));
+        return SMM_OK;
+    });
+}
+int smm_debug_plan_into(void* ctx, int which, int t, int bg) {
+    return api_call(ctx, true, [&](Ctx* c) -> int {
+        if (t < 1 || t > c->P.T || (bg && !plan_bg_fits(c->P.Ng, c->P.plan_K))) return SMM_ERR_INVALID_ARG;
+        HIPCHK(hipSetDevice(c->device));
+        const int tiles = debug_plan_sets(c);
+        if (!tiles) return SMM_ERR_INVALID_ARG;
+        if (c->pstream) HIPCHK(hipStreamSynchronize(c->pstream));
+        Ctx::PlanSet& S = c->ps[which & 1];
+        KParams Pw = c->P;
+        point_tables(Pw, S);
+        if (!c->plan_beside) { Pw.cone_tiles = tiles; Pw.cone_ct = NORM_CT; }
+        const int W = std::min(c->F.plan_cap, Pw.T - t + 1);
+        launch_exch(c, bg ? XI_PLAN_BG : XI_PLAN, dim3(W), bg ? PBG_LDS : plan_smem(Pw.Ng, Pw.plan_K, true), c->stream, Pw, t, S.plan, S.plan_mi, S.lv_pairs, S.lv_mi, S.lv_off,
+                    S.lv_pairs_p, S.lv_offp);
+        HIPCHK(hipStreamSynchronize(c->stream));
+        S.t0 = t; S.w = W;
+        if (c->plan_beside && (which & 1) == c->ps_act) { c->plan_t0 = t; c->plan_w = W; c->P.plan_t0 = t; }
+        return SMM_OK;
+    });
+}
 int smm_debug_plan_window(void* ctx, int t, double* ms_out, int* window_out) {
     return api_call(ctx, ms_out != nullptr, [&](Ctx* c) -> int {
         HIPCHK(hipSetDevice(c->device));
diff --git a/smm.jl_amd/host.py b/smm.jl_amd/host.py
--- a/smm.jl_amd/host.py
+++ b/smm.jl_amd/host.py
@@ -1053,6 +1053,10 @@
     return SobolResult(names, ms_names(m), ctx.sens_sobol(n_base, lo, hi))
 
 
+def plan_beside(algo):
+    return algo._ctx.plan_beside_info()
+
+
 def set_proposal(algo, L):
     algo._ctx.set_proposal(L)
 
```

After: 378.5 million, median of 6. +5.0%, better.
